# HongMJ1315/Path_Tracing

Hardware: AMD Instinct MI355X
Metric: Msamples/s (paths/s) at 1024^2 x 256spp (higher is better)
Workload: dtype f32; 1 GPU; configs[2]: unidirectional PT + NEE, Cornell-style box + tessellated sphere, 99024 triangles behind a BVH, 1024x1024, 256 spp, depth 4, 1 cone light; parallelism=image tiles 32x32 round-robin over 1 rank(s), RCCL gather to rank 0, seed=1

## Files before the change

### include/hpt.h

```cpp
#ifndef HPT_H
#define HPT_H

#include <stddef.h>
#include <stdint.h>

#ifdef __cplusplus
extern "C" {
#endif

#define HPT_OK 0
#define HPT_ERR_INVALID 1
#define HPT_ERR_DEVICE 2
#define HPT_ERR_NOMEM 3

#define HPT_LIGHT_BYTES 144
#define HPT_SPHERE_BYTES 100
#define HPT_TRIANGLE_BYTES 120
#define HPT_CAMERA_BYTES 84

typedef struct hpt_scene hpt_scene;

typedef struct hpt_params {
    uint64_t seed;
    int32_t sample_offset;
// ... 90 lines not shown
    uint64_t photon_rays;
    uint64_t deposits;
    uint64_t hit_points;
    uint64_t direct_pixels;
    uint64_t candidates;
    uint64_t accepted;
    uint64_t cand_median, cand_max, acc_median, acc_max;
    uint64_t grid_buckets;
    double ms_eye, ms_photon, ms_grid, ms_gather;
    double ms_total;
} hpt_ppm_stats;
int hpt_ppm_get_stats(const hpt_scene *scene, hpt_ppm_stats *out);

int hpt_ppm_render_wrapper(const void *lights, int num_lights, const void *spheres, int num_spheres,
                           const void *triangles, int num_triangles,
                           const float scene_min[3], const float scene_max[3],
                           const void *camera, float *host_image, int W, int H,
                           int light_depth, int light_sample, int eye_depth, int spp, int64_t seed);

typedef struct hpt_sppm hpt_sppm;
int hpt_sppm_create(hpt_scene *scene, const void *camera, int W, int H, int eye_depth, int light_depth, int spl,
                    float radius, float alpha, const float *scene_min, const float *scene_max,
                    const hpt_params *params, hpt_sppm **out);
int hpt_sppm_render(hpt_sppm *state, int passes, int32_t flags, float *host_image);
int hpt_sppm_reset(hpt_sppm *state);
int hpt_sppm_read_state(const hpt_sppm *state, float *radius2, float *photons, int64_t *passes);
void hpt_sppm_destroy(hpt_sppm *state);

typedef struct hpt_multi hpt_multi;
int hpt_multi_create(const void *lights, int num_lights, const void *spheres, int num_spheres,
                     const void *triangles, int num_triangles,
                     const int *device_ids, int num_devices, int exchange, hpt_multi **out);
void hpt_multi_destroy(hpt_multi *multi);
int hpt_multi_num_devices(const hpt_multi *multi);
int hpt_multi_set_groups(hpt_multi *multi, const int32_t *obj_kind, const int32_t *obj_index,
                         const int32_t *obj_group, int num_objects);
int hpt_multi_render_pt(hpt_multi *multi, const void *camera, int W, int H, int eye_depth, int spp,
                        const hpt_params *params, float *host_image);
int hpt_multi_render_bdpt(hpt_multi *multi, const void *camera, int W, int H, int eye_depth, int light_depth,
                          int spp, int spl, const hpt_params *params, float *host_image);
int hpt_multi_get_timing(const hpt_multi *multi, double *render_ms_per_device, double *gather_ms, double *total_ms);
int hpt_wrapper_set_devices(int num_devices);

int hpt_probe_functions(const float *records_in, int n, float *results_out);

int hpt_tonemap(const void *d_linear_rgb, void *d_rgb8, int64_t num_pixels, int bgr, void *hip_stream);
int hpt_tonemap_host(const float *linear_rgb, unsigned char *rgb8, int64_t num_pixels, int bgr);
void hpt_tonemap_table(float thresholds_out[256]);
void hpt_tonemap_reference(const float *linear_rgb, unsigned char *rgb8, int64_t num_pixels, int bgr);

typedef struct hpt_denoise_params {
    int32_t iterations;
    float sigma_color;
    float sigma_normal;
    float sigma_position;
    int32_t flags;
} hpt_denoise_params;
#define HPT_DENOISE_DEMODULATE 1
#define HPT_DENOISE_TIME 2

int hpt_render_guides(hpt_scene *scene, const void *camera, int W, int H, int spp,
                      const hpt_params *params,
                      float *albedo, float *normal, float *position, float *coverage);
int hpt_render_guides_device(hpt_scene *scene, const void *camera, int W, int H, int spp,
                             const hpt_params *params,
                             void *d_albedo, void *d_normal, void *d_position, void *d_coverage);

typedef struct hpt_denoiser hpt_denoiser;
int hpt_denoiser_create(int W, int H, hpt_denoiser **out);
int hpt_denoiser_set_guides(hpt_denoiser *d, const void *d_albedo, const void *d_normal,
                            const void *d_position, const void *d_coverage, void *hip_stream);
int hpt_denoiser_run(hpt_denoiser *d, const void *d_linear_rgb, void *d_out,
                     const hpt_denoise_params *p, void *hip_stream);
int hpt_denoiser_last_ms(const hpt_denoiser *d, double *ms_pack, double *ms_filter);
int hpt_denoiser_level_ms(const hpt_denoiser *d, double *ms_levels, int cap);
void hpt_denoiser_destroy(hpt_denoiser *d);
int hpt_denoise_host(const float *linear_rgb, const float *albedo, const float *normal, const float *position,
                     const float *coverage, float *out, int W, int H, const hpt_denoise_params *p);

#define HPT_ACCUM_MOMENTS 1
typedef struct hpt_accum hpt_accum;
int  hpt_accum_create(int W, int H, int32_t flags, hpt_accum **out);
int  hpt_accum_add(hpt_accum *a, const void *d_frame_rgb, void *d_mean_out, void *hip_stream);
int  hpt_accum_mean(hpt_accum *a, void *d_out, void *hip_stream);
int  hpt_accum_variance(hpt_accum *a, void *d_out, void *hip_stream);
int  hpt_accum_reset(hpt_accum *a, void *hip_stream);
int64_t hpt_accum_count(const hpt_accum *a);
int  hpt_accum_read(hpt_accum *a, float *sum, float *sumsq, int64_t *count);
void hpt_accum_destroy(hpt_accum *a);

#define HPT_DISPLAY_BGR    1
#define HPT_DISPLAY_FLIP_Y 2
typedef struct hpt_display hpt_display;
int  hpt_display_create(int W, int H, hpt_display **out);
int  hpt_display_present(hpt_display *d, const void *d_linear_rgb, const hpt_display *other,
                         void *d_rgb8, int64_t pitch_bytes, int64_t x_offset_bytes, int32_t flags, void *hip_stream);
int  hpt_display_metrics(hpt_display *d, double *rms_prev, double *rms_other,
                         uint64_t *ssd_prev, uint64_t *ssd_other, int64_t *presented);
int  hpt_display_reset(hpt_display *d, void *hip_stream);
void hpt_display_destroy(hpt_display *d);

typedef struct hpt_history hpt_history;
typedef struct hpt_history_params {
    float max_history;
    float plane_tolerance;
    float normal_min;
    int32_t flags;
} hpt_history_params;
int  hpt_history_create(int W, int H, hpt_history **out);
int  hpt_history_advance(hpt_history *h, const void *camera, const void *d_frame_rgb,
                         const void *d_normal, const void *d_position, const void *d_coverage,
                         const hpt_history_params *p, void *d_mean_out, void *hip_stream);
int  hpt_history_metrics(hpt_history *h, uint64_t *kept, uint64_t *restarted, int64_t *frames);
int  hpt_history_read(hpt_history *h, float *mean, float *length, int64_t *frames);
int  hpt_history_reset(hpt_history *h, void *hip_stream);
void hpt_history_destroy(hpt_history *h);
int  hpt_history_check(int W, int H, const void *camera, const void *d_frame_rgb,
                       const void *d_normal, const void *d_position, const void *d_coverage,
                       const hpt_history_params *p, const void *d_mean_out);

#define HPT_HISTORY_MOMENTS 1
int  hpt_history_create_flags(int W, int H, int32_t flags, hpt_history **out);
int  hpt_history_variance(hpt_history *h, const void *d_fallback, float min_length, void *d_variance_out, void *hip_stream);
int  hpt_history_read_moments(hpt_history *h, float *q);
int  hpt_history_variance_check(int W, int H, int32_t create_flags, const void *d_fallback, float min_length,
                                const void *d_variance_out);

typedef struct hpt_guided_params {
    int32_t iterations;
    float sigma_color;
    float sigma_normal;
    float sigma_position;
    int32_t flags;
} hpt_guided_params;
int hpt_denoiser_run_guided(hpt_denoiser *d, const void *d_linear_rgb, const void *d_variance,
                            void *d_out, void *d_variance_out,
                            const hpt_guided_params *p, void *hip_stream);
int hpt_denoiser_estimate_variance(hpt_denoiser *d, const void *d_frame_rgb, const void *d_length,
                                   void *d_variance_out, const hpt_guided_params *p, void *hip_stream);
int hpt_history_length(hpt_history *h, void *d_length_out, void *hip_stream);
int hpt_guided_check(int W, int H, const void *d_linear_rgb, const void *d_variance, const void *d_out,
                     const void *d_variance_out, const hpt_guided_params *p);

typedef struct hpt_bvh_info {
    int32_t num_nodes, num_tris, bvh_depth, num_rounds;
    float qorigin[3], qscale[3];
} hpt_bvh_info;
int hpt_bvh_export_host(const void *lights, int num_lights, const void *spheres, int num_spheres,
                        const void *triangles, int num_triangles, hpt_bvh_info *info,
                        void *qnodes_out, size_t qnodes_cap, void *tris_out, size_t tris_cap);
int hpt_scene_export_bvh(const hpt_scene *scene, hpt_bvh_info *info,
                         void *qnodes_out, size_t qnodes_cap, void *tris_out, size_t tris_cap);

int hpt_trace_closest(hpt_scene *scene, const float *origins, const float *dirs, int n,
                      int flags, float *t_out, int32_t *prim_out);
int hpt_trace_visibility(hpt_scene *scene, const float *p1, const float *p2, int n,
                         int flags, int32_t *visible_out);

typedef struct hpt_update_info {
    uint64_t updates, live_tris, dead_tris;
    double ms_pack, ms_upload, ms_refit;
} hpt_update_info;
int hpt_scene_update_triangles(hpt_scene *scene, const void *triangles, int num_triangles);
int hpt_scene_update_rounds(hpt_scene *scene, const void *lights, int num_lights, const void *spheres, int num_spheres);
int hpt_scene_update_check(const hpt_scene *scene, const void *triangles, int num_triangles);
int hpt_scene_get_update_info(const hpt_scene *scene, hpt_update_info *out);
int hpt_bvh_refit_host(const void *lights, int num_lights, const void *spheres, int num_spheres, const void *triangles,
                       const void *new_triangles, int num_triangles, hpt_bvh_info *info,
                       void *qnodes_out, size_t qnodes_cap, void *tris_out, size_t tris_cap);

#ifdef __cplusplus
}
#endif
#endif
```

### path_tracing_amd/__init__.py

```python
from __future__ import annotations

import ctypes as C
import os

import numpy as np

from . import layouts, scene_io
from .layouts import CAMERA, LIGHT, SPHERE, TRIANGLE

_HERE = os.path.dirname(os.path.abspath(__file__))
LIB_PATH = os.path.join(_HERE, "csrc", "libhpt.so")

FLAG_BRUTE_FORCE = 1
FLAG_COUNT_WORK = 2
FLAG_OUTPUT_SUM = 4
FLAG_TIME_KERNELS = 8
FLAG_RUSSIAN_ROULETTE = 16
FLAG_SINGLE_PIPELINE = 32
FLAG_NO_HOST_WAIT = 64
DENOISE_DEMODULATE = 1
DENOISE_TIME = 2
ACCUM_MOMENTS = 1
DISPLAY_BGR = 1
DISPLAY_FLIP_Y = 2
HISTORY_MOMENTS = 1


class HptError(RuntimeError):
    pass


class Params(C.Structure):
    _fields_ = [("seed", C.c_uint64), ("sample_offset", C.c_int32), ("max_delta", C.c_int32),
                ("rank", C.c_int32), ("world", C.c_int32), ("tile", C.c_int32),
                ("samples_per_pass", C.c_int32), ("flags", C.c_int32), ("reserved", C.c_int32)]


class Stats(C.Structure):
    _fields_ = [("samples", C.c_uint64), ("closest_rays", C.c_uint64), ("shadow_rays", C.c_uint64),
                ("boxes_closest", C.c_uint64), ("tris_closest", C.c_uint64),
                ("boxes_shadow", C.c_uint64), ("tris_shadow", C.c_uint64), ("path_iters", C.c_uint64),
                ("ms_total", C.c_double), ("ms_extend", C.c_double), ("ms_shade", C.c_double),
                ("ms_connect", C.c_double), ("ms_other", C.c_double),
                ("n_extend", C.c_uint32), ("n_shade", C.c_uint32), ("n_connect", C.c_uint32), ("n_other", C.c_uint32),
                ("bvh_nodes", C.c_uint32), ("bvh_depth", C.c_uint32), ("n_tris", C.c_uint32), ("n_materials", C.c_uint32),
                ("ms_bvh_build", C.c_double), ("ms_upload", C.c_double),
                ("lane_steps_closest", C.c_uint64), ("wave_steps_closest", C.c_uint64),
                ("lane_steps_shadow", C.c_uint64), ("wave_steps_shadow", C.c_uint64),
                ("leaf_lane_closest", C.c_uint64), ("leaf_wave_closest", C.c_uint64),
                ("leaf_lane_shadow", C.c_uint64), ("leaf_wave_shadow", C.c_uint64),
                ("ms_resume", C.c_double), ("n_resume", C.c_uint32), ("split_budget", C.c_uint32),
                ("traced_rays_last_pass", C.c_uint64), ("long_rays_last_pass", C.c_uint64),
                ("bd_pairs", C.c_uint64), ("bd_survivors", C.c_uint64), ("bd_shadow_rays", C.c_uint64), ("bd_unoccluded", C.c_uint64),
                ("bd_nodes", C.c_uint64), ("bd_tris", C.c_uint64), ("bd_spheres", C.c_uint64), ("bd_group_boxes", C.c_uint64)]

    def as_dict(self):
        return {n: getattr(self, n) for n, _ in self._fields_}


class PpmStats(C.Structure):
    _fields_ = [(n, C.c_uint64) for n in ("photons", "photon_rays", "deposits", "hit_points", "direct_pixels", "candidates", "accepted",
                                          "cand_median", "cand_max", "acc_median", "acc_max", "grid_buckets")] + \
               [(n, C.c_double) for n in ("ms_eye", "ms_photon", "ms_grid", "ms_gather", "ms_total")]

    def as_dict(self):
        return {n: getattr(self, n) for n, _ in self._fields_}


class DenoiseParams(C.Structure):
    _fields_ = [("iterations", C.c_int32), ("sigma_color", C.c_float), ("sigma_normal", C.c_float),
                ("sigma_position", C.c_float), ("flags", C.c_int32)]


class GuidedParams(C.Structure):
    _fields_ = [("iterations", C.c_int32), ("sigma_color", C.c_float), ("sigma_normal", C.c_float),
                ("sigma_position", C.c_float), ("flags", C.c_int32)]


class HistoryParams(C.Structure):
    _fields_ = [("max_history", C.c_float), ("plane_tolerance", C.c_float), ("normal_min", C.c_float), ("flags", C.c_int32)]


def make_history_params(max_history=0.0, plane_tolerance=0.0, normal_min=0.0) -> HistoryParams:
    return HistoryParams(float(max_history), float(plane_tolerance), float(normal_min), 0)


def make_denoise_params(iterations=0, sigma_color=0.0, sigma_normal=0.0, sigma_position=0.0, demodulate=True, time=False) -> DenoiseParams:
    return DenoiseParams(int(iterations), float(sigma_color), float(sigma_normal), float(sigma_position),
                         (DENOISE_DEMODULATE if demodulate else 0) | (DENOISE_TIME if time else 0))


def make_guided_params(iterations=0, sigma_color=0.0, sigma_normal=0.0, sigma_position=0.0, demodulate=True, time=False) -> GuidedParams:
    return GuidedParams(int(iterations), float(sigma_color), float(sigma_normal), float(sigma_position),
                        (DENOISE_DEMODULATE if demodulate else 0) | (DENOISE_TIME if time else 0))


class BvhInfo(C.Structure):
    _fields_ = [("num_nodes", C.c_int32), ("num_tris", C.c_int32), ("bvh_depth", C.c_int32), ("num_rounds", C.c_int32),
                ("qorigin", C.c_float * 3), ("qscale", C.c_float * 3)]


class UpdateInfo(C.Structure):
    _fields_ = [("updates", C.c_uint64), ("live_tris", C.c_uint64), ("dead_tris", C.c_uint64),
                ("ms_pack", C.c_double), ("ms_upload", C.c_double), ("ms_refit", C.c_double)]


QNODE_WORDS = 8
TRI_WORDS = 12

_lib = None


def _share_the_hip_runtime_with_torch():
    import importlib.util
    import sys
    if "torch" in sys.modules:
        return
    try:
        spec = importlib.util.find_spec("torch")
    except (ImportError, ValueError):
        spec = None
    if spec and spec.origin:
        cand = os.path.join(os.path.dirname(spec.origin), "lib", "libamdhip64.so")
        if os.path.exists(cand):
            C.CDLL(cand, mode=C.RTLD_GLOBAL)


def load_library() -> C.CDLL:
    global _lib
    if _lib is None:
        _share_the_hip_runtime_with_torch()
        path = os.environ.get("HPT_LIBRARY") or LIB_PATH
        if not os.path.exists(path):
            raise HptError("%s not built: run `make -C path_tracing_amd/csrc` "
                           "(or __graft_entry__.build()); there is no CPU fallback" % path)
        lib = C.CDLL(path)
        lib.hpt_last_error.restype = C.c_char_p
        lib.hpt_local_pixels.restype = C.c_int64
        lib.hpt_local_pixels.argtypes = [C.c_int, C.c_int, C.POINTER(Params)]
        for name in ("hpt_scene_create", "hpt_render_pt", "hpt_render_pt_device", "hpt_untile", "hpt_scene_set_groups",
                     "hpt_render_bdpt", "hpt_render_bdpt_device", "hpt_bdpt_render_wrapper",
                     "hpt_pt_render_wrapper", "hpt_get_stats", "hpt_trace_closest", "hpt_trace_visibility",
                     "hpt_device_count", "hpt_multi_create", "hpt_multi_num_devices", "hpt_multi_set_groups",
                     "hpt_multi_render_pt", "hpt_multi_render_bdpt", "hpt_multi_get_timing", "hpt_wrapper_set_devices",
                     "hpt_probe_functions", "hpt_tonemap", "hpt_tonemap_host", "hpt_bvh_export_host", "hpt_scene_export_bvh",
                     "hpt_render_ppm", "hpt_ppm_get_stats", "hpt_ppm_render_wrapper",
                     "hpt_sppm_create", "hpt_sppm_render", "hpt_sppm_reset", "hpt_sppm_read_state",
                     "hpt_render_guides", "hpt_denoiser_create", "hpt_denoiser_set_guides", "hpt_denoiser_run",
                     "hpt_denoiser_last_ms", "hpt_denoiser_level_ms", "hpt_denoise_host",
                     "hpt_accum_create", "hpt_accum_add", "hpt_accum_mean", "hpt_accum_variance", "hpt_accum_reset", "hpt_accum_read",
                     "hpt_display_create", "hpt_display_present", "hpt_display_metrics", "hpt_display_reset",
                     "hpt_render_guides_device", "hpt_history_create", "hpt_history_advance", "hpt_history_metrics",
                     "hpt_history_read", "hpt_history_reset", "hpt_history_check",
                     "hpt_denoiser_run_guided", "hpt_denoiser_estimate_variance", "hpt_history_length", "hpt_guided_check",
                     "hpt_history_create_flags", "hpt_history_variance", "hpt_history_read_moments", "hpt_history_variance_check",
                     "hpt_scene_update_triangles", "hpt_scene_update_rounds", "hpt_scene_update_check", "hpt_scene_get_update_info",
                     "hpt_bvh_refit_host"):
            if hasattr(lib, name):
                getattr(lib, name).restype = C.c_int
        if hasattr(lib, "hpt_sppm_destroy"):
            lib.hpt_sppm_destroy.restype = None
            lib.hpt_sppm_destroy.argtypes = [C.c_void_p]
        if hasattr(lib, "hpt_denoiser_destroy"):
            lib.hpt_denoiser_destroy.restype = None
            lib.hpt_denoiser_destroy.argtypes = [C.c_void_p]
        for name in ("hpt_accum_destroy", "hpt_display_destroy", "hpt_history_destroy"):
            if hasattr(lib, name):
                getattr(lib, name).restype = None
                getattr(lib, name).argtypes = [C.c_void_p]
        if hasattr(lib, "hpt_accum_count"):
            lib.hpt_accum_count.restype = C.c_int64
            lib.hpt_accum_count.argtypes = [C.c_void_p]
        lib.hpt_scene_destroy.restype = None
        lib.hpt_wrapper_cache_clear.restype = None
        lib.hpt_wrapper_cache_clear.argtypes = []
        lib.hpt_scene_destroy.argtypes = [C.c_void_p]
        lib.hpt_multi_destroy.restype = None
        lib.hpt_multi_destroy.argtypes = [C.c_void_p]
        _lib = lib
    return _lib


def _check(rc: int):
    if rc != 0:
        raise HptError("hpt error %d: %s" % (rc, load_library().hpt_last_error().decode("utf-8", "replace")))


def _vp(a):
    return a.ctypes.data_as(C.c_void_p) if a is not None and a.size else None


def device_count() -> int:
    return int(load_library().hpt_device_count())


def make_params(seed=1, sample_offset=0, max_delta=0, rank=0, world=1, tile=0, samples_per_pass=0, flags=0) -> Params:
    p = Params()
    p.seed, p.sample_offset, p.max_delta = int(seed), int(sample_offset), int(max_delta)
    p.rank, p.world, p.tile, p.samples_per_pass, p.flags, p.reserved = rank, world, tile, samples_per_pass, flags, 0
    return p


def local_pixels(W: int, H: int, params: Params) -> int:
    n = int(load_library().hpt_local_pixels(W, H, C.byref(params)))
    if n < 0:
        _check(1)
    return n


class Scene:

    def __init__(self, lights, spheres, triangles):
        self._lib = load_library()
        self._h = C.c_void_p()
        lights = np.ascontiguousarray(lights, LIGHT)
        spheres = np.ascontiguousarray(spheres, SPHERE)
        triangles = np.ascontiguousarray(triangles, TRIANGLE)
        _check(self._lib.hpt_scene_create(_vp(lights), len(lights), _vp(spheres), len(spheres),
                                          _vp(triangles), len(triangles), C.byref(self._h)))
        self.num_lights, self.num_spheres, self.num_triangles = len(lights), len(spheres), len(triangles)

    def close(self):
        if getattr(self, "_h", None) is not None and self._h:
            self._lib.hpt_scene_destroy(self._h)
            self._h = C.c_void_p()

    def __del__(self):
        try:
            self.close()
        except Exception:
            pass

    def __enter__(self):
        return self

    def __exit__(self, *exc):
        self.close()

    def render_pt(self, camera, W, H, eye_depth=4, spp=8, params: Params | None = None) -> np.ndarray:
        params = params or make_params()
        cam = np.ascontiguousarray(camera, CAMERA)
        img = np.empty((H, W, 3), np.float32)
        _check(self._lib.hpt_render_pt(self._h, _vp(cam.reshape(1)), W, H, eye_depth, spp, C.byref(params), _vp(img)))
        return img

    def render_pt_device(self, camera, W, H, eye_depth, spp, params: Params, d_local_ptr: int, stream: int = 0):
        cam = np.ascontiguousarray(camera, CAMERA)
        _check(self._lib.hpt_render_pt_device(self._h, _vp(cam.reshape(1)), W, H, eye_depth, spp, C.byref(params),
                                              C.c_void_p(d_local_ptr), C.c_void_p(stream)))

    def set_groups(self, kind, index, group):
        k = np.ascontiguousarray(kind, np.int32); i = np.ascontiguousarray(index, np.int32); g = np.ascontiguousarray(group, np.int32)
        _check(self._lib.hpt_scene_set_groups(self._h, _vp(k), _vp(i), _vp(g), len(k)))

    def render_bdpt(self, camera, W, H, eye_depth=4, light_depth=4, spp=8, spl=8, params: Params | None = None) -> np.ndarray:
        params = params or make_params()
        cam = np.ascontiguousarray(camera, CAMERA)
        img = np.empty((H, W, 3), np.float32)
        _check(self._lib.hpt_render_bdpt(self._h, _vp(cam.reshape(1)), W, H, eye_depth, light_depth, spp, spl, C.byref(params), _vp(img)))
        return img

    def render_bdpt_device(self, camera, W, H, eye_depth, light_depth, spp, spl, params: Params, d_local_ptr: int, stream: int = 0):
        cam = np.ascontiguousarray(camera, CAMERA)
        _check(self._lib.hpt_render_bdpt_device(self._h, _vp(cam.reshape(1)), W, H, eye_depth, light_depth, spp, spl, C.byref(params),
                                                C.c_void_p(d_local_ptr), C.c_void_p(stream)))

    def render_ppm(self, camera, W, H, eye_depth=4, light_depth=4, spp=1, spl=8, radius=0.05, params: Params | None = None,
                   scene_min=None, scene_max=None) -> np.ndarray:
        params = params or make_params()
        cam = np.ascontiguousarray(camera, CAMERA)
        img = np.empty((H, W, 3), np.float32)
        mn = (C.c_float * 3)(*scene_min) if scene_min is not None else None
        mx = (C.c_float * 3)(*scene_max) if scene_max is not None else None
        _check(self._lib.hpt_render_ppm(self._h, _vp(cam.reshape(1)), W, H, eye_depth, light_depth, spp, spl, C.c_float(radius),
                                        mn, mx, C.byref(params), _vp(img)))
        return img

    def ppm_stats(self) -> dict:
        st = PpmStats()
        _check(self._lib.hpt_ppm_get_stats(self._h, C.byref(st)))
        return st.as_dict()

    def sppm(self, camera, W, H, eye_depth=4, light_depth=4, spl=8, radius=0.05, alpha=0.7, params: Params | None = None,
             scene_min=None, scene_max=None) -> "Sppm":
        return Sppm(self, camera, W, H, eye_depth, light_depth, spl, radius, alpha, params, scene_min, scene_max)

    def render_guides(self, camera, W, H, spp=4, params: Params | None = None) -> dict:
        params = params or make_params()
        cam = np.ascontiguousarray(camera, CAMERA)
        g = dict(albedo=np.empty((H, W, 3), np.float32), normal=np.empty((H, W, 3), np.float32),
                 position=np.empty((H, W, 3), np.float32), coverage=np.empty((H, W), np.float32))
        _check(self._lib.hpt_render_guides(self._h, _vp(cam.reshape(1)), W, H, int(spp), C.byref(params), _vp(g["albedo"]),
                                           _vp(g["normal"]), _vp(g["position"]), _vp(g["coverage"])))
        return g

    def render_guides_device(self, camera, W, H, spp=4, params: Params | None = None, albedo=None, normal=None, position=None,
                             coverage=None):
        params = params or make_params()
        cam = np.ascontiguousarray(camera, CAMERA)
        ptr = [_dptr(x) if x is not None else None for x in (albedo, normal, position, coverage)]
        _check(self._lib.hpt_render_guides_device(self._h, _vp(cam.reshape(1)), W, H, int(spp), C.byref(params), *ptr))

    def stats(self) -> dict:
        st = Stats()
        _check(self._lib.hpt_get_stats(self._h, C.byref(st)))
        return st.as_dict()

    def export_bvh(self) -> dict:
        return _export_bvh(lambda info, qn, qcap, tr, tcap: self._lib.hpt_scene_export_bvh(self._h, info, qn, qcap, tr, tcap))

# ... 253 lines not shown
    def __init__(self, W, H, moments=False):
        self._lib = load_library()
        self._h = C.c_void_p()
        self.W, self.H, self.moments = int(W), int(H), bool(moments)
        if moments:
            _check(self._lib.hpt_history_create_flags(int(W), int(H), C.c_int32(HISTORY_MOMENTS), C.byref(self._h)))
        else:
            _check(self._lib.hpt_history_create(int(W), int(H), C.byref(self._h)))

    def advance(self, camera, frame, normal=None, position=None, coverage=None, params: HistoryParams | None = None, mean_out=None,
                stream: int = 0):
        cam = np.ascontiguousarray(camera, CAMERA)
        opt = [_dptr(x) if x is not None else None for x in (normal, position, coverage)]
        _check(self._lib.hpt_history_advance(self._h, _vp(cam.reshape(1)), _dptr(frame), opt[0], opt[1], opt[2],
                                             C.byref(params) if params is not None else None,
                                             _dptr(mean_out) if mean_out is not None else None, C.c_void_p(stream)))

    def metrics(self) -> dict:
        k, r = C.c_uint64(), C.c_uint64()
        n = C.c_int64()
        _check(self._lib.hpt_history_metrics(self._h, C.byref(k), C.byref(r), C.byref(n)))
        return dict(kept=int(k.value), restarted=int(r.value), frames=int(n.value))

    def read(self) -> dict:
        m = np.empty((self.H, self.W, 3), np.float32)
        n = np.empty((self.H, self.W), np.float32)
        k = C.c_int64()
        _check(self._lib.hpt_history_read(self._h, _vp(m), _vp(n), C.byref(k)))
        out = dict(mean=m, length=n, frames=int(k.value))
        if self.moments:
            q = np.empty((self.H, self.W, 3), np.float32)
            _check(self._lib.hpt_history_read_moments(self._h, _vp(q)))
            out["q"] = q
        return out

    def variance(self, out, fallback=None, min_length=0.0, stream: int = 0):
        _check(self._lib.hpt_history_variance(self._h, _dptr(fallback) if fallback is not None else None, C.c_float(min_length),
                                              _dptr(out) if out is not None else None, C.c_void_p(stream)))

    def length(self, out, stream: int = 0):
        _check(self._lib.hpt_history_length(self._h, _dptr(out), C.c_void_p(stream)))

    def reset(self, stream: int = 0):
        _check(self._lib.hpt_history_reset(self._h, C.c_void_p(stream)))

    def close(self):
        if getattr(self, "_h", None) is not None and self._h:
            self._lib.hpt_history_destroy(self._h)
            self._h = C.c_void_p()

    def __del__(self):
        try:
            self.close()
        except Exception:
            pass

    def __enter__(self):
        return self

    def __exit__(self, *exc):
        self.close()


class MultiScene:

    def __init__(self, lights, spheres, triangles, device_ids=None, num_devices=0, exchange=0):
        self._lib = load_library()
        self._h = C.c_void_p()
        lights = np.ascontiguousarray(lights, LIGHT)
        spheres = np.ascontiguousarray(spheres, SPHERE)
        triangles = np.ascontiguousarray(triangles, TRIANGLE)
        ids = None
        if device_ids is not None:
            ids = np.ascontiguousarray(device_ids, np.int32)
            num_devices = len(ids)
        _check(self._lib.hpt_multi_create(_vp(lights), len(lights), _vp(spheres), len(spheres), _vp(triangles), len(triangles),
                                          _vp(ids), int(num_devices), int(exchange), C.byref(self._h)))
        self.num_devices = int(self._lib.hpt_multi_num_devices(self._h))

    def close(self):
        if getattr(self, "_h", None) is not None and self._h:
            self._lib.hpt_multi_destroy(self._h)
            self._h = C.c_void_p()

    def __del__(self):
        try:
            self.close()
        except Exception:
            pass

    def __enter__(self):
        return self

    def __exit__(self, *exc):
        self.close()

    def set_groups(self, kind, index, group):
        k = np.ascontiguousarray(kind, np.int32); i = np.ascontiguousarray(index, np.int32); g = np.ascontiguousarray(group, np.int32)
        _check(self._lib.hpt_multi_set_groups(self._h, _vp(k), _vp(i), _vp(g), len(k)))

    def render_pt(self, camera, W, H, eye_depth=4, spp=8, params: Params | None = None) -> np.ndarray:
        params = params or make_params()
        cam = np.ascontiguousarray(camera, CAMERA)
        img = np.empty((H, W, 3), np.float32)
        _check(self._lib.hpt_multi_render_pt(self._h, _vp(cam.reshape(1)), W, H, eye_depth, spp, C.byref(params), _vp(img)))
        return img

    def render_bdpt(self, camera, W, H, eye_depth=4, light_depth=4, spp=8, spl=8, params: Params | None = None) -> np.ndarray:
        params = params or make_params()
        cam = np.ascontiguousarray(camera, CAMERA)
        img = np.empty((H, W, 3), np.float32)
        _check(self._lib.hpt_multi_render_bdpt(self._h, _vp(cam.reshape(1)), W, H, eye_depth, light_depth, spp, spl, C.byref(params), _vp(img)))
        return img

    def timing(self) -> dict:
        per = (C.c_double * self.num_devices)()
        g = C.c_double(); t = C.c_double()
        _check(self._lib.hpt_multi_get_timing(self._h, per, C.byref(g), C.byref(t)))
        return {"render_ms_per_device": list(per), "gather_ms": g.value, "total_ms": t.value}


def _export_bvh(call) -> dict:
    info = BvhInfo()
    _check(call(C.byref(info), None, C.c_size_t(0), None, C.c_size_t(0)))
    qn = np.zeros((max(info.num_nodes, 1), QNODE_WORDS), np.uint32)
    tr = np.zeros((max(info.num_tris, 1), TRI_WORDS), np.uint32)
    _check(call(C.byref(info), _vp(qn), C.c_size_t(qn.nbytes), _vp(tr), C.c_size_t(tr.nbytes)))
    return {"num_nodes": info.num_nodes, "num_tris": info.num_tris, "bvh_depth": info.bvh_depth, "num_rounds": info.num_rounds,
            "qorigin": np.array(info.qorigin, np.float32), "qscale": np.array(info.qscale, np.float32),
            "qnodes": qn[:info.num_nodes], "tris": tr[:info.num_tris]}


def export_bvh_host(lights, spheres, triangles) -> dict:
    lib = load_library()
    lights = np.ascontiguousarray(lights, LIGHT)
    spheres = np.ascontiguousarray(spheres, SPHERE)
    triangles = np.ascontiguousarray(triangles, TRIANGLE)
    return _export_bvh(lambda info, qn, qcap, tr, tcap: lib.hpt_bvh_export_host(
        _vp(lights), len(lights), _vp(spheres), len(spheres), _vp(triangles), len(triangles), info, qn, qcap, tr, tcap))


def refit_bvh_host(lights, spheres, triangles, new_triangles) -> dict:
    lib = load_library()
    lights = np.ascontiguousarray(lights, LIGHT)
    spheres = np.ascontiguousarray(spheres, SPHERE)
    triangles = np.ascontiguousarray(triangles, TRIANGLE)
    new_triangles = np.ascontiguousarray(new_triangles, TRIANGLE)
    if len(new_triangles) != len(triangles):
        raise HptError("hpt error 1: an update keeps the triangle count: %d triangles, %d were handed over" % (len(triangles), len(new_triangles)))
    return _export_bvh(lambda info, qn, qcap, tr, tcap: lib.hpt_bvh_refit_host(
        _vp(lights), len(lights), _vp(spheres), len(spheres), _vp(triangles), _vp(new_triangles), len(triangles), info, qn, qcap, tr, tcap))


def update_check(scene, triangles, num_triangles=None) -> None:
    tr = np.ascontiguousarray(triangles, TRIANGLE) if triangles is not None else None
    n = len(tr) if num_triangles is None else int(num_triangles)
    _check(load_library().hpt_scene_update_check(scene._h if scene is not None else None, _vp(tr) if tr is not None else None, n))


def probe_functions(records) -> np.ndarray:
    rec = np.ascontiguousarray(records, np.float32).reshape(-1, 24)
    out = np.zeros((len(rec), 40), np.float32)
    _check(load_library().hpt_probe_functions(_vp(rec), len(rec), _vp(out)))
    return out


def tonemap(image) -> np.ndarray:
    img = np.ascontiguousarray(image, np.float32)
    out = np.zeros(img.shape, np.uint8)
    _check(load_library().hpt_tonemap_host(_vp(img), _vp(out), C.c_int64(img.size // 3), 0))
    return out


def tonemap_device(d_linear_rgb, d_rgb8, num_pixels: int, bgr: bool = False, stream: int = 0):
    _check(load_library().hpt_tonemap(_dptr(d_linear_rgb), _dptr(d_rgb8), C.c_int64(num_pixels), 1 if bgr else 0, C.c_void_p(stream)))


def wrapper_set_devices(n: int) -> None:
    _check(load_library().hpt_wrapper_set_devices(int(n)))


def untile(d_gathered_ptr: int, d_image_ptr: int, W: int, H: int, params: Params, stream: int = 0):
    _check(load_library().hpt_untile(C.c_void_p(d_gathered_ptr), C.c_void_p(d_image_ptr), W, H, C.byref(params), C.c_void_p(stream)))


def wrapper_cache_clear() -> None:
    load_library().hpt_wrapper_cache_clear()


def pt_render_wrapper(lights, spheres, triangles, camera, W, H, eye_depth, spp, seed=-1,
                      scene_min=(0, 0, 0), scene_max=(0, 0, 0), light_depth=4, light_sample=8) -> np.ndarray:
    lib = load_library()
    lights = np.ascontiguousarray(lights, LIGHT)
    spheres = np.ascontiguousarray(spheres, SPHERE)
    triangles = np.ascontiguousarray(triangles, TRIANGLE)
    cam = np.ascontiguousarray(camera, CAMERA).reshape(1)
    img = np.empty((H, W, 3), np.float32)
    mn = (C.c_float * 3)(*scene_min)
    mx = (C.c_float * 3)(*scene_max)
    _check(lib.hpt_pt_render_wrapper(_vp(lights), len(lights), _vp(spheres), len(spheres), _vp(triangles), len(triangles),
                                     mn, mx, _vp(cam), _vp(img), W, H, light_depth, light_sample, eye_depth, spp,
                                     C.c_int64(seed)))
    return img


def ppm_render_wrapper(lights, spheres, triangles, camera, W, H, scene_min, scene_max, light_depth=4, light_sample=8,
                       eye_depth=4, spp=1, seed=-1) -> np.ndarray:
    lib = load_library()
    lights = np.ascontiguousarray(lights, LIGHT)
    spheres = np.ascontiguousarray(spheres, SPHERE)
    triangles = np.ascontiguousarray(triangles, TRIANGLE)
    cam = np.ascontiguousarray(camera, CAMERA).reshape(1)
    img = np.empty((H, W, 3), np.float32)
    mn = (C.c_float * 3)(*scene_min)
    mx = (C.c_float * 3)(*scene_max)
    _check(lib.hpt_ppm_render_wrapper(_vp(lights), len(lights), _vp(spheres), len(spheres), _vp(triangles), len(triangles),
                                      mn, mx, _vp(cam), _vp(img), W, H, light_depth, light_sample, eye_depth, spp, C.c_int64(seed)))
    return img
```

### path_tracing_amd/csrc/hpt_api.cpp

```cpp
#include "hpt_host.h"

#include <chrono>
#include <cmath>
#include <cstdio>
#include <cstdlib>
#include <ctime>
#include <mutex>
#include <new>

using namespace hpt;

static_assert(sizeof(hpt_stats) == 312 && sizeof(hpt_params) == 40, "ABI records: keep path_tracing_amd/__init__.py and tests/test_boundary.py in step");

namespace {

thread_local std::string g_err;

}

namespace hpt {

int fail(int code, const std::string &msg){ g_err = msg; return code; }

int make_tiling(int W, int H, const hpt_params *p, Tiling &tl){
// ... 43 lines not shown
    HIP_TRY(s->ws.local_own.reserve((size_t) tl.n_local * 3));
    HIP_TRY(s->ws.image_own.reserve((size_t) tl.W * tl.H * 3));
    return HPT_OK;
}

int untile_to_host(hpt_scene *s, const Tiling &tl, hipStream_t st, float *host_image, hipEvent_t after){
    launch_untile(st, tl, s->ws.local_own.get(), s->ws.image_own.get());
    if(after) HIP_TRY(hipEventRecord(after, st));
    HIP_TRY(hipGetLastError());
    HIP_TRY(hipMemcpy(host_image, s->ws.image_own.get(), (size_t) tl.W * tl.H * 3 * sizeof(float), hipMemcpyDeviceToHost));
    return HPT_OK;
}

}

namespace {

int collect_stats(hpt_scene *s){
    if(!s->tm.stats_pending) return HPT_OK;
    HIP_TRY(hipEventSynchronize(s->tm.ev_stop));
    float ms = 0.f;
    HIP_TRY(hipEventElapsedTime(&ms, s->tm.ev_start, s->tm.ev_stop));
    s->tm.stats.ms_total = ms;
    double sum[5] = { 0, 0, 0, 0, 0 }; uint32_t cnt[5] = { 0, 0, 0, 0, 0 };
    for(const TimedLaunch &t : s->tm.timed){
        float e = 0.f;
        if(hipEventElapsedTime(&e, t.a, t.b) == hipSuccess){ sum[t.cls] += e; cnt[t.cls]++; }
    }
    s->tm.stats.ms_extend = sum[0]; s->tm.stats.ms_shade = sum[1]; s->tm.stats.ms_connect = sum[2]; s->tm.stats.ms_other = sum[3];
    s->tm.stats.n_extend = cnt[0]; s->tm.stats.n_shade = cnt[1]; s->tm.stats.n_connect = cnt[2]; s->tm.stats.n_other = cnt[3];
    s->tm.stats.ms_resume = sum[4]; s->tm.stats.n_resume = cnt[4];
    s->tm.stats.split_budget = (uint32_t) s->ws.last_budget;
    s->tm.stats.traced_rays_last_pass = s->tm.stats.long_rays_last_pass = 0;
    if(s->ws.last_counter_stride > 0 && s->ws.last_counters){
        std::vector<uint32_t> h((size_t) 4 * s->ws.last_counter_stride);
        HIP_TRY(hipMemcpy(h.data(), s->ws.last_counters, h.size() * sizeof(uint32_t), hipMemcpyDeviceToHost));
        for(int i = 0; i < s->ws.last_counter_stride; ++i){
            s->tm.stats.traced_rays_last_pass += (uint64_t) h[i] + h[(size_t) s->ws.last_counter_stride + i];
            s->tm.stats.long_rays_last_pass += (uint64_t) h[(size_t) 2 * s->ws.last_counter_stride + i] + h[(size_t) 3 * s->ws.last_counter_stride + i];
        }
    }
    WorkCounters wc;
    HIP_TRY(hipMemcpy(&wc, s->ws.wc.get(), sizeof wc, hipMemcpyDeviceToHost));
    s->tm.stats.samples = wc.samples; s->tm.stats.closest_rays = wc.closest_rays; s->tm.stats.shadow_rays = wc.shadow_rays;
    s->tm.stats.boxes_closest = wc.boxes_closest; s->tm.stats.tris_closest = wc.tris_closest;
    s->tm.stats.boxes_shadow = wc.boxes_shadow; s->tm.stats.tris_shadow = wc.tris_shadow; s->tm.stats.path_iters = wc.path_iters;
    s->tm.stats.lane_steps_closest = wc.lane_steps_closest; s->tm.stats.wave_steps_closest = wc.wave_steps_closest;
    s->tm.stats.lane_steps_shadow = wc.lane_steps_shadow; s->tm.stats.wave_steps_shadow = wc.wave_steps_shadow;
    s->tm.stats.leaf_lane_closest = wc.leaf_lane_closest; s->tm.stats.leaf_wave_closest = wc.leaf_wave_closest;
    s->tm.stats.leaf_lane_shadow = wc.leaf_lane_shadow; s->tm.stats.leaf_wave_shadow = wc.leaf_wave_shadow;
    s->tm.stats.bd_pairs = wc.bd_pairs; s->tm.stats.bd_survivors = wc.bd_survivors; s->tm.stats.bd_shadow_rays = wc.bd_shadow_rays;
    s->tm.stats.bd_unoccluded = wc.bd_unoccluded; s->tm.stats.bd_nodes = wc.bd_nodes; s->tm.stats.bd_tris = wc.bd_tris;
    s->tm.stats.bd_spheres = wc.bd_spheres; s->tm.stats.bd_group_boxes = wc.bd_group_boxes;
    s->tm.stats_pending = false;
    return HPT_OK;
}

struct WrapperCache { std::mutex mu; hpt_scene *scene = nullptr; int device = -1; hpt_multi *multi = nullptr; int devices = 0; } g_wrap;

bool wrapper_cache_enabled(){
    static const bool on = [](){ const char *e = getenv("HPT_WRAPPER_CACHE"); return !(e && e[0] == '0'); }();
    return on;
}

int wrapper_devices(){
    if(g_wrap.devices > 0) return g_wrap.devices;
    static const int from_env = [](){ const char *e = getenv("HPT_DEVICES"); int v = e ? atoi(e) : 1; return v > 0 ? v : 1; }();
    return from_env;
}

int wrapper_scene(const void *lights, int nl, const void *spheres, int ns, const void *tris, int nt, hpt_scene **out){
    int dev = -1;
    if(hipGetDevice(&dev) != hipSuccess) dev = -1;
    hpt_scene *k = g_wrap.scene;
    if(k && wrapper_cache_enabled() && dev == g_wrap.device && nl == k->geo.nl && ns == k->geo.ns && nt == k->geo.nt && nl >= 0 && ns >= 0 && nt >= 0 &&
       same_bytes(k->geo.h_lights, lights, (size_t) nl * HPT_LIGHT_BYTES) && same_bytes(k->geo.h_spheres, spheres, (size_t) ns * HPT_SPHERE_BYTES) &&
       same_bytes(k->geo.h_tris, tris, (size_t) nt * HPT_TRIANGLE_BYTES)){
        *out = k;
        return HPT_OK;
    }
    if(k){ hpt_scene_destroy(k); g_wrap.scene = nullptr; g_wrap.device = -1; }
    int rc = hpt_scene_create(lights, nl, spheres, ns, tris, nt, out);
    if(rc) return rc;
    if(wrapper_cache_enabled()){ g_wrap.scene = *out; g_wrap.device = dev; }
    return HPT_OK;
}

void wrapper_release(hpt_scene *s){
    if(s == g_wrap.scene) return;
    std::string keep = g_err;
    hpt_scene_destroy(s);
    g_err = keep;
}

int wrapper_multi(int devices, const void *lights, int nl, const void *spheres, int ns, const void *tris, int nt, hpt_multi **out){
    if(g_wrap.multi && wrapper_cache_enabled() && hpt::multi_matches(g_wrap.multi, devices, lights, nl, spheres, ns, tris, nt)){
        *out = g_wrap.multi;
        return HPT_OK;
    }
    if(g_wrap.multi){ hpt_multi_destroy(g_wrap.multi); g_wrap.multi = nullptr; }
    int rc = hpt_multi_create(lights, nl, spheres, ns, tris, nt, nullptr, devices, 0, out);
    if(rc) return rc;
    if(wrapper_cache_enabled()) g_wrap.multi = *out;
    return HPT_OK;
}

void wrapper_release_multi(hpt_multi *m){
    if(m == g_wrap.multi) return;
    std::string keep = g_err;
    hpt_multi_destroy(m);
    g_err = keep;
}

hpt_params wrapper_params(int64_t seed){
    hpt_params p; memset(&p, 0, sizeof p);
    p.seed = seed >= 0 ? (uint64_t) seed : (uint64_t) time(nullptr);
    return p;
}

template <typename One, typename Many>
int wrapper_render(const void *lights, int nl, const void *spheres, int ns, const void *tris, int nt, One one, Many many){
    std::lock_guard<std::mutex> lock(g_wrap.mu);
    if(wrapper_devices() > 1){
        hpt_multi *m = nullptr;
        int rc = wrapper_multi(wrapper_devices(), lights, nl, spheres, ns, tris, nt, &m);
        if(rc) return rc;
        rc = many(m);
        wrapper_release_multi(m);
        return rc;
    }
    hpt_scene *s = nullptr;
    int rc = wrapper_scene(lights, nl, spheres, ns, tris, nt, &s);
    if(rc) return rc;
    rc = one(s);
    wrapper_release(s);
    return rc;
}

}

namespace hpt {

int scene_upload(const HostScene &hs, const void *lights, int nl, const void *spheres, int ns, const void *tris, int nt,
                 hpt_scene **out){
    *out = nullptr;
    hpt_scene *s = new (std::nothrow) hpt_scene();
    if(!s) return fail(HPT_ERR_NOMEM, "out of host memory");
    auto t0 = std::chrono::steady_clock::now();
    hipError_t e = hipGetDevice(&s->device);
    if(e == hipSuccess){ hipDeviceProp_t prop; if(hipGetDeviceProperties(&prop, s->device) == hipSuccess && prop.multiProcessorCount > 0) s->num_cus = prop.multiProcessorCount; }
    if(e == hipSuccess) e = s->geo.nodes.upload(hs.nodes);
    if(e == hipSuccess) e = s->geo.qnodes.upload(hs.qnodes);
    if(e == hipSuccess) e = s->geo.wnodes.upload(hs.wnodes);
    if(e == hipSuccess) e = s->geo.tris.upload(hs.tris);
    if(e == hipSuccess) e = s->geo.rounds.upload(hs.rounds);
    if(e == hipSuccess) e = s->geo.mats.upload(hs.materials);
    if(e == hipSuccess) e = s->geo.lights.upload(hs.lights);
    if(e != hipSuccess){ hpt_scene_destroy(s); return fail_hip("scene upload", e); }
    e = s->geo.tri_frames.reserve(std::max<size_t>((size_t) nt, 1) * 4);
    if(e == hipSuccess){
        launch_tri_frames(nullptr, (const float4 *) s->geo.tris.get(), nt, s->geo.tri_frames.get());
        e = hipDeviceSynchronize();
    }
    if(e != hipSuccess){ hpt_scene_destroy(s); return fail_hip("triangle frames", e); }
    auto t1 = std::chrono::steady_clock::now();
    s->geo.sd.nodes = (const float4 *) s->geo.nodes.get(); s->geo.sd.tris = (const float4 *) s->geo.tris.get();
    s->geo.sd.tri_frames = s->geo.tri_frames.get();
    s->geo.sd.qnodes = (const uint4 *) s->geo.qnodes.get();
    s->geo.sd.wnodes = (const uint4 *) s->geo.wnodes.get(); s->geo.sd.wide_depth = hs.wide_depth;
    for(int a = 0; a < 3; ++a){ s->geo.sd.qorigin[a] = hs.qorigin[a]; s->geo.sd.qscale[a] = hs.qscale[a]; }
    s->geo.sd.rounds = s->geo.rounds.get(); s->geo.sd.mats = s->geo.mats.get(); s->geo.sd.lights = s->geo.lights.get();
    s->geo.sd.num_rounds = ns + nl; s->geo.sd.num_spheres = ns; s->geo.sd.num_lights = nl; s->geo.sd.num_tris = nt;
    s->geo.sd.num_mats = (int) hs.materials.size(); s->geo.sd.num_nodes = (int) hs.qnodes.size();
    s->geo.nl = nl; s->geo.ns = ns; s->geo.nt = nt;
    if(nl) s->geo.h_lights.assign((const unsigned char *) lights, (const unsigned char *) lights + (size_t) nl * HPT_LIGHT_BYTES);
    if(ns) s->geo.h_spheres.assign((const unsigned char *) spheres, (const unsigned char *) spheres + (size_t) ns * HPT_SPHERE_BYTES);
    if(nt) s->geo.h_tris.assign((const unsigned char *) tris, (const unsigned char *) tris + (size_t) nt * HPT_TRIANGLE_BYTES);
    memset(&s->tm.stats, 0, sizeof s->tm.stats);
    s->tm.stats.bvh_nodes = (uint32_t) hs.nodes.size(); s->tm.stats.bvh_depth = (uint32_t) hs.bvh_depth;
    s->geo.stack_levels = hs.bvh_depth > 0 ? hs.bvh_depth : 1;
    s->tm.stats.n_tris = (uint32_t) nt; s->tm.stats.n_materials = (uint32_t) hs.materials.size();
    s->tm.stats.ms_bvh_build = hs.ms_bvh_build;
    s->tm.stats.ms_upload = std::chrono::duration<double, std::milli>(t1 - t0).count();
    s->up.level_begin = hs.level_begin; s->up.wide_src = hs.wide_src; s->up.num_wide = (uint32_t) hs.wnodes.size();
    s->up.sphere_material.resize((size_t) ns);
    for(int i = 0; i < ns; ++i) s->up.sphere_material[(size_t) i] = hs.rounds[(size_t) i].material;
    *out = s;
    return HPT_OK;
}

int export_host_tree(const HostScene &hs, hpt_bvh_info *info, void *qnodes_out, size_t qnodes_cap, void *tris_out, size_t tris_cap){
    info->num_nodes = (int32_t) hs.qnodes.size(); info->num_tris = (int32_t) hs.tris.size();
    info->bvh_depth = hs.bvh_depth; info->num_rounds = hs.num_spheres + hs.num_lights;
    for(int a = 0; a < 3; ++a){ info->qorigin[a] = hs.qorigin[a]; info->qscale[a] = hs.qscale[a]; }
    if(qnodes_out){
        if(qnodes_cap < hs.qnodes.size() * sizeof(QBvhNode)) return fail(HPT_ERR_INVALID, "qnodes_out too small");
        memcpy(qnodes_out, hs.qnodes.data(), hs.qnodes.size() * sizeof(QBvhNode));
    }
    if(tris_out){
        if(tris_cap < hs.tris.size() * sizeof(DevTriangle)) return fail(HPT_ERR_INVALID, "tris_out too small");
        memcpy(tris_out, hs.tris.data(), hs.tris.size() * sizeof(DevTriangle));
    }
    return HPT_OK;
}

}

extern "C" {

const char *hpt_last_error(void){ return g_err.c_str(); }

int hpt_device_count(void){
    int n = 0;
    if(hipGetDeviceCount(&n) != hipSuccess) return -1;
    return n;
}

int hpt_scene_create(const void *lights, int nl, const void *spheres, int ns, const void *tris, int nt,
                     hpt_scene **out){
    if(!out) return fail(HPT_ERR_INVALID, "null out_scene");
    *out = nullptr;
    HostScene hs;
    const char *err = build_host_scene(lights, nl, spheres, ns, tris, nt, hs);
    if(err && *err) return fail(HPT_ERR_INVALID, err);
    return hpt::scene_upload(hs, lights, nl, spheres, ns, tris, nt, out);
}

void hpt_scene_destroy(hpt_scene *s){
    if(!s) return;
    for(PassBuffers &w : s->ws.pass) if(w.h_count) hipHostFree(w.h_count);
    if(s->ws.px_fork) hipEventDestroy(s->ws.px_fork);
    for(int k = 1; k < kMaxPipes; ++k){
        if(s->ws.px_done[k]) hipEventDestroy(s->ws.px_done[k]);
        if(s->ws.px_stream[k]) hipStreamDestroy(s->ws.px_stream[k]);
    }
    for(hipEvent_t e : s->pm.marks) hipEventDestroy(e);
    if(s->up.ev_a) hipEventDestroy(s->up.ev_a);
    if(s->up.ev_b) hipEventDestroy(s->up.ev_b);
    if(s->tm.ev_start) hipEventDestroy(s->tm.ev_start);
    if(s->tm.ev_stop) hipEventDestroy(s->tm.ev_stop);
    for(hipEvent_t e : s->tm.event_pool) hipEventDestroy(e);
    delete s;
}

int64_t hpt_local_pixels(int W, int H, const hpt_params *params){
    Tiling tl;
    if(make_tiling(W, H, params, tl)) return -1;
    return tl.n_local;
}

int hpt_untile(const void *d_gathered, void *d_image, int W, int H, const hpt_params *params, void *hip_stream){
    Tiling tl;
    int rc = make_tiling(W, H, params, tl);
    if(rc) return rc;
    if(!d_gathered || !d_image) return fail(HPT_ERR_INVALID, "null buffer");
    launch_untile((hipStream_t) hip_stream, tl, (const float *) d_gathered, (float *) d_image);
    HIP_TRY(hipGetLastError());
    return HPT_OK;
}


void hpt_wrapper_cache_clear(void){
    std::lock_guard<std::mutex> lock(g_wrap.mu);
    if(g_wrap.scene) hpt_scene_destroy(g_wrap.scene);
    g_wrap.scene = nullptr; g_wrap.device = -1;
    if(g_wrap.multi) hpt_multi_destroy(g_wrap.multi);
    g_wrap.multi = nullptr;
}

int hpt_wrapper_set_devices(int num_devices){
    if(num_devices < 0) return fail(HPT_ERR_INVALID, "negative device count");
    std::lock_guard<std::mutex> lock(g_wrap.mu);
    g_wrap.devices = num_devices;
    return HPT_OK;
}

int hpt_pt_render_wrapper(const void *lights, int nl, const void *spheres, int ns, const void *tris, int nt,
                          const float scene_min[3], const float scene_max[3], const void *camera, float *host_image,
                          int W, int H, int light_depth, int light_sample, int eye_depth, int spp, int64_t seed){
    (void) scene_min; (void) scene_max; (void) light_depth; (void) light_sample;
    const hpt_params p = wrapper_params(seed);
    return wrapper_render(lights, nl, spheres, ns, tris, nt,
        [&](hpt_scene *s){ return hpt_render_pt(s, camera, W, H, eye_depth, spp, &p, host_image); },
        [&](hpt_multi *m){ return hpt_multi_render_pt(m, camera, W, H, eye_depth, spp, &p, host_image); });
}

namespace {

unsigned char tonemap_byte(float x){
    float c = std::max(0.0f, std::min(x, 1.0f));
    float g = std::pow(c, 1.0f / 2.2f);
    return (unsigned char) (g * 255.0f);
}

const float *tonemap_thresholds(){
    static float table[256];
    static std::once_flag once;
    std::call_once(once, [](){
        table[0] = -INFINITY;
        for(int k = 1; k < 256; ++k){
            uint32_t lo = 0u, hi = 0x3F800000u;
            while(lo < hi){
                uint32_t mid = lo + (hi - lo) / 2u;
                float x; memcpy(&x, &mid, 4);
                if((int) tonemap_byte(x) >= k) hi = mid; else lo = mid + 1u;
            }
            memcpy(&table[k], &lo, 4);
        }
    });
    return table;
}

struct TonemapDevice { std::mutex mu; DevBuf<float> table[64]; } &g_tonemap = *new TonemapDevice;

int tonemap_device_table(const float **out){
    int dev = 0;
    HIP_TRY(hipGetDevice(&dev));
    if(dev < 0 || dev >= 64) return fail(HPT_ERR_INVALID, "device ordinal out of range");
    std::lock_guard<std::mutex> lock(g_tonemap.mu);
    DevBuf<float> &d = g_tonemap.table[dev];
    if(!d.get()){
        HIP_TRY(d.reserve(256));
        hipError_t e = hipMemcpy(d.get(), tonemap_thresholds(), 256 * sizeof(float), hipMemcpyHostToDevice);
        if(e != hipSuccess){ d.release(); return fail(HPT_ERR_DEVICE, std::string("tonemap table upload: ") + hipGetErrorString(e)); }
    }
    *out = d.get();
    return HPT_OK;
}

}

void hpt_tonemap_table(float thresholds_out[256]){ memcpy(thresholds_out, tonemap_thresholds(), 256 * sizeof(float)); }

void hpt_tonemap_reference(const float *linear_rgb, unsigned char *rgb8, int64_t num_pixels, int bgr){
    for(int64_t p = 0; p < num_pixels; ++p)
        for(int c = 0; c < 3; ++c) rgb8[p * 3 + c] = tonemap_byte(linear_rgb[p * 3 + (bgr ? 2 - c : c)]);
}

int hpt_tonemap(const void *d_linear_rgb, void *d_rgb8, int64_t num_pixels, int bgr, void *hip_stream){
    if(num_pixels < 0 || (num_pixels > 0 && (!d_linear_rgb || !d_rgb8))) return fail(HPT_ERR_INVALID, "bad tonemap argument");
    if(((uintptr_t) d_rgb8 & 3u) != 0u) return fail(HPT_ERR_INVALID, "tonemap output must be 4-byte aligned");
    const float *table = nullptr;
    int rc = tonemap_device_table(&table);
    if(rc) return rc;
    launch_tonemap((hipStream_t) hip_stream, (const float *) d_linear_rgb, d_rgb8, (unsigned long long) num_pixels * 3ull, bgr ? 1 : 0, table);
    HIP_TRY(hipGetLastError());
    return HPT_OK;
}

int hpt_tonemap_host(const float *linear_rgb, unsigned char *rgb8, int64_t num_pixels, int bgr){
    if(num_pixels < 0 || (num_pixels > 0 && (!linear_rgb || !rgb8))) return fail(HPT_ERR_INVALID, "bad tonemap argument");
    if(num_pixels == 0) return HPT_OK;
    DevBuf<float> d_in; DevBuf<unsigned char> d_out;
    size_t n = (size_t) num_pixels * 3;
    HIP_TRY(d_in.reserve(n));
    HIP_TRY(d_out.reserve((n + 3) / 4 * 4));
    HIP_TRY(hipMemcpy(d_in.get(), linear_rgb, n * sizeof(float), hipMemcpyHostToDevice));
    int rc = hpt_tonemap(d_in.get(), d_out.get(), num_pixels, bgr, nullptr);
    if(rc) return rc;
    HIP_TRY(hipMemcpy(rgb8, d_out.get(), n, hipMemcpyDeviceToHost));
    return HPT_OK;
}

int hpt_get_stats(const hpt_scene *scene, hpt_stats *out){
    if(!scene || !out) return fail(HPT_ERR_INVALID, "null argument");
    int rc = collect_stats(const_cast<hpt_scene *>(scene));
    if(rc) return rc;
    *out = scene->tm.stats;
    return HPT_OK;
}

int hpt_trace_closest(hpt_scene *s, const float *origins, const float *dirs, int n, int flags,
                      float *t_out, int32_t *prim_out){
    if(!s || !origins || !dirs || !t_out || !prim_out || n < 0) return fail(HPT_ERR_INVALID, "bad argument");
    if(n == 0) return HPT_OK;
    DevBuf<float> d_o, d_d, d_t; DevBuf<int32_t> d_p;
    size_t b3 = (size_t) n * 3 * sizeof(float);
    HIP_TRY(d_o.reserve((size_t) n * 3)); HIP_TRY(d_d.reserve((size_t) n * 3));
    HIP_TRY(d_t.reserve((size_t) n)); HIP_TRY(d_p.reserve((size_t) n));
    HIP_TRY(hipMemcpy(d_o.get(), origins, b3, hipMemcpyHostToDevice));
    HIP_TRY(hipMemcpy(d_d.get(), dirs, b3, hipMemcpyHostToDevice));
    launch_probe_closest(nullptr, s->geo.sd, d_o.get(), d_d.get(), n, (flags & HPT_FLAG_BRUTE_FORCE) ? 1 : 0, d_t.get(), d_p.get());
    HIP_TRY(hipGetLastError());
    HIP_TRY(hipMemcpy(t_out, d_t.get(), (size_t) n * 4, hipMemcpyDeviceToHost));
    HIP_TRY(hipMemcpy(prim_out, d_p.get(), (size_t) n * 4, hipMemcpyDeviceToHost));
    return HPT_OK;
}

int hpt_probe_functions(const float *records_in, int n, float *results_out){
    if(n < 0 || (n > 0 && (!records_in || !results_out))) return fail(HPT_ERR_INVALID, "bad argument");
    if(n == 0) return HPT_OK;
    DevBuf<float> d_in, d_out;
    HIP_TRY(d_in.reserve((size_t) n * 24));
    HIP_TRY(d_out.reserve((size_t) n * 40));
    HIP_TRY(hipMemcpy(d_in.get(), records_in, (size_t) n * 24 * sizeof(float), hipMemcpyHostToDevice));
    launch_probe_functions(nullptr, d_in.get(), n, d_out.get());
    HIP_TRY(hipGetLastError());
    HIP_TRY(hipMemcpy(results_out, d_out.get(), (size_t) n * 40 * sizeof(float), hipMemcpyDeviceToHost));
    return HPT_OK;
}

int hpt_scene_set_groups(hpt_scene *s, const int32_t *obj_kind, const int32_t *obj_index, const int32_t *obj_group, int nobj){
    if(!s) return fail(HPT_ERR_INVALID, "null scene");
    if(nobj < 0 || (nobj > 0 && (!obj_kind || !obj_index || !obj_group))) return fail(HPT_ERR_INVALID, "bad group arrays");
    if(nobj != 0 && nobj != s->geo.ns + s->geo.nt) return fail(HPT_ERR_INVALID, "group arrays must list every sphere and triangle once");
    s->geo.g_kind.assign(obj_kind, obj_kind + nobj); s->geo.g_index.assign(obj_index, obj_index + nobj); s->geo.g_group.assign(obj_group, obj_group + nobj);
    s->bd.ready = false;
    return HPT_OK;
}


int hpt_bdpt_render_wrapper(const void *lights, int nl, const void *spheres, int ns, const void *tris, int nt,
                            const float scene_min[3], const float scene_max[3], const void *camera, float *host_image,
                            int W, int H, int light_depth, int light_sample, int eye_depth, int spp, int spl, int64_t seed){
    (void) scene_min; (void) scene_max;
    std::vector<unsigned char> L((const unsigned char *) lights, (const unsigned char *) lights + (size_t) std::max(nl, 0) * HPT_LIGHT_BYTES);
    if(light_sample > 1) for(int i = 0; i < nl; ++i){
        float *illum = (float *) (L.data() + (size_t) i * HPT_LIGHT_BYTES + 24);
        for(int c = 0; c < 3; ++c) illum[c] = illum[c] * (float) light_sample;
    }
    const hpt_params p = wrapper_params(seed);
    return wrapper_render(L.data(), nl, spheres, ns, tris, nt,
        [&](hpt_scene *s){ return hpt_render_bdpt(s, camera, W, H, eye_depth, light_depth, spp, spl, &p, host_image); },
        [&](hpt_multi *m){ return hpt_multi_render_bdpt(m, camera, W, H, eye_depth, light_depth, spp, spl, &p, host_image); });
}

int hpt_ppm_render_wrapper(const void *lights, int nl, const void *spheres, int ns, const void *tris, int nt,
                           const float scene_min[3], const float scene_max[3], const void *camera, float *host_image,
                           int W, int H, int light_depth, int light_sample, int eye_depth, int spp, int64_t seed){
    (void) spp;
    std::lock_guard<std::mutex> lock(g_wrap.mu);
    hpt_scene *s = nullptr;
    int rc = wrapper_scene(lights, nl, spheres, ns, tris, nt, &s);
    if(rc) return rc;
    const hpt_params p = wrapper_params(seed);
    rc = hpt_render_ppm(s, camera, W, H, eye_depth, light_depth, 1, light_sample, 0.05f, scene_min, scene_max, &p, host_image);
    wrapper_release(s);
    return rc;
}

int hpt_bvh_export_host(const void *lights, int nl, const void *spheres, int ns, const void *tris, int nt, hpt_bvh_info *info,
                        void *qnodes_out, size_t qnodes_cap, void *tris_out, size_t tris_cap){
    if(!info) return fail(HPT_ERR_INVALID, "null info");
    HostScene hs;
    const char *err = build_host_scene(lights, nl, spheres, ns, tris, nt, hs);
    if(err && *err) return fail(HPT_ERR_INVALID, err);
    return export_host_tree(hs, info, qnodes_out, qnodes_cap, tris_out, tris_cap);
}

int hpt_scene_export_bvh(const hpt_scene *s, hpt_bvh_info *info, void *qnodes_out, size_t qnodes_cap, void *tris_out, size_t tris_cap){
    if(!s || !info) return fail(HPT_ERR_INVALID, "null argument");
    if(int rcd = on_scene_device(s)) return rcd;
    info->num_nodes = s->geo.sd.num_nodes; info->num_tris = s->geo.sd.num_tris;
    info->bvh_depth = (int32_t) s->tm.stats.bvh_depth; info->num_rounds = s->geo.sd.num_rounds;
    for(int a = 0; a < 3; ++a){ info->qorigin[a] = s->geo.sd.qorigin[a]; info->qscale[a] = s->geo.sd.qscale[a]; }
    if(qnodes_out){
        const size_t bytes = (size_t) s->geo.sd.num_nodes * sizeof(QBvhNode);
        if(qnodes_cap < bytes) return fail(HPT_ERR_INVALID, "qnodes_out too small");
        HIP_TRY(hipMemcpy(qnodes_out, s->geo.qnodes.get(), bytes, hipMemcpyDeviceToHost));
    }
    if(tris_out){
        const size_t bytes = (size_t) s->geo.sd.num_tris * sizeof(DevTriangle);
        if(tris_cap < bytes) return fail(HPT_ERR_INVALID, "tris_out too small");
        if(bytes) HIP_TRY(hipMemcpy(tris_out, s->geo.tris.get(), bytes, hipMemcpyDeviceToHost));
    }
    return HPT_OK;
}

int hpt_trace_visibility(hpt_scene *s, const float *p1, const float *p2, int n, int flags, int32_t *vis_out){
    if(!s || !p1 || !p2 || !vis_out || n < 0) return fail(HPT_ERR_INVALID, "bad argument");
    if(n == 0) return HPT_OK;
    DevBuf<float> d_a, d_b; DevBuf<int32_t> d_v;
    size_t b3 = (size_t) n * 3 * sizeof(float);
    HIP_TRY(d_a.reserve((size_t) n * 3)); HIP_TRY(d_b.reserve((size_t) n * 3));
    HIP_TRY(d_v.reserve((size_t) n));
    HIP_TRY(hipMemcpy(d_a.get(), p1, b3, hipMemcpyHostToDevice));
    HIP_TRY(hipMemcpy(d_b.get(), p2, b3, hipMemcpyHostToDevice));
    launch_probe_visibility(nullptr, s->geo.sd, d_a.get(), d_b.get(), n, (flags & HPT_FLAG_BRUTE_FORCE) ? 1 : 0, d_v.get());
    HIP_TRY(hipGetLastError());
    HIP_TRY(hipMemcpy(vis_out, d_v.get(), (size_t) n * 4, hipMemcpyDeviceToHost));
    return HPT_OK;
}

}
```

### path_tracing_amd/csrc/hpt_host.h

```cpp
#pragma once
#include "../../include/hpt.h"
#include "hpt_scene.h"
#include "pt_kernels.h"
#include "bdpt_kernels.h"
#include "ppm_kernels.h"
#include "denoise_kernels.h"
#include "refit_kernels.h"

#include <hip/hip_runtime.h>
#include <algorithm>
#include <cstring>
#include <string>
#include <vector>

namespace hpt {

int fail(int code, const std::string &msg);

inline int fail_hip(const std::string &what, hipError_t e){
    return fail(e == hipErrorOutOfMemory ? HPT_ERR_NOMEM : HPT_ERR_DEVICE, what + ": " + hipGetErrorString(e));
}

#define HIP_TRY(expr) do { hipError_t e_ = (expr); if(e_ != hipSuccess) return hpt::fail_hip(#expr, e_); } while(0)

template <typename T>
class DevBuf {
    T *p_ = nullptr; size_t cap_ = 0;
public:
    DevBuf() = default;
    DevBuf(const DevBuf &) = delete;
    DevBuf &operator=(const DevBuf &) = delete;
    ~DevBuf(){ release(); }
    T *get() const { return p_; }
    size_t capacity() const { return cap_; }
    void release(){ if(p_) hipFree(p_); p_ = nullptr; cap_ = 0; }
    hipError_t reserve(size_t n){
        if(n <= cap_) return hipSuccess;
        release();
        hipError_t e = hipMalloc((void **) &p_, n * sizeof(T));
        if(e != hipSuccess){ p_ = nullptr; return e; }
        cap_ = n;
        return hipSuccess;
    }
    template <typename A>
    hipError_t upload(const std::vector<T, A> &v){
        release();
        hipError_t e = reserve(std::max<size_t>(v.size(), 1));
        if(e == hipSuccess && !v.empty()) e = hipMemcpy(p_, v.data(), v.size() * sizeof(T), hipMemcpyHostToDevice);
        return e;
    }
};

template <typename First, typename... Rest>
hipError_t reserve_all(size_t n, First &first, Rest &... rest){
    if(n <= first.capacity()) return hipSuccess;
    first.release(); (rest.release(), ...);
    hipError_t e = first.reserve(n);
    ((e = e == hipSuccess ? rest.reserve(n) : e), ...);
    if(e != hipSuccess){ first.release(); (rest.release(), ...); }
    return e;
}

struct TimedLaunch { hipEvent_t a, b; int cls; };
constexpr int kMaxPipes = 2;

}

struct hpt_scene {
    int device = 0;
    int num_cus = 256;

    struct Geometry {
        hpt::SceneDev sd{};
        hpt::DevBuf<hpt::BvhNode> nodes; hpt::DevBuf<hpt::QBvhNode> qnodes; hpt::DevBuf<hpt::WideNode> wnodes;
        hpt::DevBuf<hpt::DevTriangle> tris; hpt::DevBuf<hpt::DevRound> rounds;
        hpt::DevBuf<hpt::DevMaterial> mats; hpt::DevBuf<hpt::DevLight> lights;
        hpt::DevBuf<float4> tri_frames;
        int stack_levels = hpt::kStackDepth;
        std::vector<unsigned char> h_lights, h_spheres, h_tris;
        int nl = 0, ns = 0, nt = 0;
        std::vector<int32_t> g_kind, g_index, g_group;
    } geo;

    struct PassBuffers {
        hpt::DevBuf<float4> org_eta, dir_flags, thr, col; hpt::DevBuf<uint2> rng, hit;
        hpt::DevBuf<float4> org_max, dir, contrib;
        hpt::PathBuf pb{}; hpt::ShadowBuf sb{};
        hpt::DevBuf<uint32_t> queue[2];
        hpt::DevBuf<uint32_t> squeue;
        hpt::DevBuf<uint32_t> lqueue[2];
        hpt::DevBuf<hpt::DeferredRay> rec;
        hpt::DevBuf<uint32_t> deep_stack;
        hpt::DevBuf<uint32_t> counters;
        uint32_t *h_count = nullptr;
        size_t cap_paths() const { return org_eta.capacity(); }
    };
    struct Workspace {
        PassBuffers pass[hpt::kMaxPipes];
        hipStream_t px_stream[hpt::kMaxPipes] = {}; int px_priority[hpt::kMaxPipes] = {};
        hipEvent_t px_fork = nullptr, px_done[hpt::kMaxPipes] = {};
        const uint32_t *last_counters = nullptr;
        int last_counter_stride = 0;
        int last_budget = 0;
        hpt::DevBuf<float4> accum;
        hpt::DevBuf<hpt::WorkCounters> wc;
        hpt::DevBuf<float> local_own, image_own;
    } ws;

    struct Bdpt {
        bool ready = false;
        hpt::BdptSceneDev sc{};
        hpt::DevBuf<hpt::BvhNode> nodes; hpt::DevBuf<hpt::DevTriangle> tris; hpt::DevBuf<hpt::DevRound> spheres;
        hpt::DevBuf<hpt::DevGroup> groups; hpt::DevBuf<hpt::DevMaterial> mats; hpt::DevBuf<hpt::DevLight> lights;
        hpt::DevBuf<float4> last_pos_pdf, last_normal, vtx_pos, vtx_nrm, vtx_thr, vtx_wo, vtx_base, ectx, hist_pos_eta, contrib;
        hpt::DevBuf<float2> hist_pdf; hpt::DevBuf<unsigned long long> valid;
        hpt::BdptPathBuf bp{};
        hpt::DevBuf<hpt::LightVertexDev> lv; hpt::DevBuf<hpt::LightVertexCtx> lctx; hpt::DevBuf<uint32_t> cqueue;
    } bd;

    struct Ppm {
        bool bounds_ready = false; float min[3] = {0, 0, 0}, max[3] = {0, 0, 0};
        hpt::DevBuf<float4> pos_mat, nrm, wo, thr; hpt::DevBuf<uint32_t> list;
        hpt::DevBuf<float4> dep, packed; hpt::DevBuf<uint32_t> key, slot_in, key_sorted, slot_sorted;
        hpt::DevBuf<uint2> range; hpt::DevBuf<unsigned char> sort_tmp;
        hpt::PpmHitBuf hb{}; hpt::PpmGrid grid{};
        hpt::DevBuf<uint32_t> cand, acc;
        hpt::DevBuf<hpt::PpmCounters> pc;
        hpt::DevBuf<float4> g_alb, g_nrm, g_pos;
        std::vector<hipEvent_t> marks;
        hpt_ppm_stats stats{};
    } pm;

    struct Update {
        std::vector<uint32_t> level_begin;
        hpt::pod_vector<uint32_t> wide_src;
        std::vector<uint32_t> sphere_material;
        uint32_t num_wide = 0;
        bool ready = false;
        hpt::DevBuf<uint4> d_wide_src;
        hpt::DevBuf<float> verts, slot_box, exact, partial, result;
        std::vector<float> h_verts;
        hipEvent_t ev_a = nullptr, ev_b = nullptr;
        hpt_update_info info{};
    } up;

    struct Timing {
        hipEvent_t ev_start = nullptr, ev_stop = nullptr;
        std::vector<hpt::TimedLaunch> timed; std::vector<hipEvent_t> event_pool; size_t event_next = 0;
        hpt_stats stats{};
        bool stats_pending = false;
    } tm;
};

namespace hpt {

using PassBuffers = hpt_scene::PassBuffers;


int on_scene_device(const hpt_scene *s);

struct ParamRules {
    const char *one_device;
    int32_t flags; const char *flags_msg;
    int32_t reserved; const char *reserved_msg;
};
constexpr int32_t kKnownFlags = HPT_FLAG_BRUTE_FORCE | HPT_FLAG_COUNT_WORK | HPT_FLAG_OUTPUT_SUM | HPT_FLAG_TIME_KERNELS |
                                HPT_FLAG_RUSSIAN_ROULETTE | HPT_FLAG_SINGLE_PIPELINE | HPT_FLAG_NO_HOST_WAIT;
constexpr int32_t kReservedBudgetBits = 0x3F << 1;
constexpr ParamRules kRenderParams{ nullptr, kKnownFlags, nullptr, kReservedBudgetBits, nullptr };
int take_params(const hpt_params *params, const ParamRules &rules, hpt_params &P);

int make_tiling(int W, int H, const hpt_params *p, Tiling &tl);

inline void set_camera(CameraDev &cam, const void *camera){
    const float *cf = (const float *) camera;
    memcpy(cam.eye, cf + 0, 12); memcpy(cam.UL, cf + 12, 12); memcpy(cam.dx, cf + 15, 12); memcpy(cam.dy, cf + 18, 12);
}

int ensure_workspace(hpt_scene *s, size_t paths, size_t n_local, int n_counters);

int ensure_own_image(hpt_scene *s, const Tiling &tl);
int untile_to_host(hpt_scene *s, const Tiling &tl, hipStream_t st, float *host_image, hipEvent_t after = nullptr);

inline void reset_render_stats(hpt_scene *s){
    s->tm.timed.clear(); s->tm.event_next = 0;
    s->ws.last_counter_stride = 0; s->ws.last_budget = 0;
    s->tm.stats.ms_total = s->tm.stats.ms_extend = s->tm.stats.ms_shade = s->tm.stats.ms_connect = s->tm.stats.ms_other = 0.0;
    s->tm.stats.n_extend = s->tm.stats.n_shade = s->tm.stats.n_connect = s->tm.stats.n_other = 0;
}

inline hipEvent_t pool_event(hpt_scene *s){
    if(s->tm.event_next == s->tm.event_pool.size()){
        hipEvent_t e; hipEventCreate(&e); s->tm.event_pool.push_back(e);
    }
    return s->tm.event_pool[s->tm.event_next++];
}

struct LaunchTimer {
    hpt_scene *s; hipStream_t st; bool on; TimedLaunch tl;
    LaunchTimer(hpt_scene *s_, hipStream_t st_, bool on_, int cls) : s(s_), st(st_), on(on_) {
        if(on){ tl.a = pool_event(s); tl.b = pool_event(s); tl.cls = cls; hipEventRecord(tl.a, st); }
    }
    ~LaunchTimer(){ if(on){ hipEventRecord(tl.b, st); s->tm.timed.push_back(tl); } }
};

inline bool same_bytes(const std::vector<unsigned char> &kept, const void *given, size_t bytes){
    return kept.size() == bytes && (bytes == 0 || memcmp(kept.data(), given, bytes) == 0);
}

int export_host_tree(const HostScene &hs, hpt_bvh_info *info, void *qnodes_out, size_t qnodes_cap, void *tris_out, size_t tris_cap);

bool multi_matches(const hpt_multi *m, int n_devices, const void *lights, int nl, const void *spheres, int ns, const void *tris, int nt);

}
```

### path_tracing_amd/csrc/hpt_scene.h

```cpp
#pragma once
#include <cstdint>
#include <memory>
#include <utility>
#include <vector>

namespace hpt {

constexpr uint32_t kLeafFlag = 0x80000000u;
constexpr uint32_t kEmptyChild = 0xFFFFFFFFu;
constexpr int kMaxLeafTris = 2;
constexpr int kMaxBvhDepth = 30;
constexpr int kStackDepth = 32;

struct Float4 { float x, y, z, w; };

template <typename T>
struct default_init_allocator : std::allocator<T> {
    template <typename U> struct rebind { using other = default_init_allocator<U>; };
    default_init_allocator() = default;
    template <typename U> default_init_allocator(const default_init_allocator<U> &){}
    template <typename U> void construct(U *p){ ::new((void *) p) U; }
    template <typename U, typename... A> void construct(U *p, A &&... a){ ::new((void *) p) U(std::forward<A>(a)...); }
};
template <typename T> using pod_vector = std::vector<T, default_init_allocator<T>>;

struct BvhNode {
    float lmin[3]; uint32_t left;
    float lmax[3]; uint32_t right;
    float rmin[3]; uint32_t pad0;
    float rmax[3]; uint32_t pad1;
};

struct QBvhNode {
    uint16_t plane[3][2][2];
    uint32_t left, right;
};

struct WideNode { uint32_t w[16]; };

struct DevTriangle {
    float v0[3]; uint32_t ordinal;
    float e1[3]; uint32_t material;
    float e2[3]; uint32_t flags;
};

struct DevRound {
    float c[3]; float r;
    uint32_t material;
    uint32_t flags;
    uint32_t pad[2];
};

struct DevMaterial {
    float base[3]; float roughness;
    float metallic; float eta; uint32_t type; uint32_t pad;
    float diffuse[3]; float pad2;
};

struct DevLight {
    float pos[3]; float r;
    float main_dir[3]; float cos_cutoff;
    float neg_dir[3]; float cutoff;
    float illum[3]; float area;
    uint32_t is_parallel; float cone_ratio;
    uint32_t pad[2];
    float raw_dir[3]; uint32_t pad2;
    float ball_c[3]; uint32_t pad3;
};

static_assert(sizeof(BvhNode) == 64 && sizeof(DevTriangle) == 48 && sizeof(DevRound) == 32, "layout");
static_assert(sizeof(QBvhNode) == 32 && sizeof(WideNode) == 64, "layout");
static_assert(sizeof(DevMaterial) == 48 && sizeof(DevLight) == 112, "layout");

struct HostScene {
    pod_vector<BvhNode> nodes;
    pod_vector<QBvhNode> qnodes;
    pod_vector<WideNode> wnodes;
    int wide_depth = 0;
    pod_vector<uint32_t> wide_src;
    std::vector<uint32_t> level_begin;
    float qorigin[3] = {0, 0, 0}, qscale[3] = {1, 1, 1};
    pod_vector<DevTriangle> tris;
    std::vector<DevRound> rounds;
    std::vector<DevMaterial> materials;
    std::vector<DevLight> lights;
    int num_spheres = 0, num_lights = 0, num_tris = 0;
    int bvh_depth = 0;
    double ms_bvh_build = 0.0;
};

struct DevGroup {
    float mn[3]; uint32_t root;
    float mx[3]; uint32_t sphere_first;
    uint32_t sphere_count; uint32_t pad[3];
};
static_assert(sizeof(DevGroup) == 48, "layout");

struct HostBdptScene {
    std::vector<BvhNode> nodes;
    std::vector<DevTriangle> tris;
    std::vector<DevRound> spheres;
    std::vector<DevGroup> groups;
    std::vector<DevMaterial> materials;
    std::vector<DevLight> lights;
    float scene_min[3], scene_max[3];
    int bvh_depth = 0;
};

const char *build_bdpt_host_scene(const void *lights, int nl, const void *spheres, int ns, const void *tris, int nt,
                                  const int32_t *obj_kind, const int32_t *obj_index, const int32_t *obj_group, int nobj,
                                  HostBdptScene &out);

const char *build_host_scene(const void *lights, int nl, const void *spheres, int ns,
                             const void *tris, int nt, HostScene &out);


const char *flatten_rounds_host(const void *lights, int nl, const void *spheres, int ns, const uint32_t *sphere_material,
                                std::vector<DevRound> &rounds, std::vector<DevLight> &lights_out);

const char *check_triangle_update(const void *kept, int kept_nt, const void *tris, int nt, char *msg, size_t msg_cap);
const char *check_rounds_update(const void *kept_spheres, int kept_ns, int kept_nl, const void *lights, int nl, const void *spheres, int ns,
                                char *msg, size_t msg_cap);

const char *refit_host_scene(HostScene &hs, const void *tris, int nt, uint64_t *dead_out = nullptr);

float box_padding_of(const float scene_min[3], const float scene_max[3], int nt);
void grid_of_box(const float lo[3], const float hi[3], float qorigin[3], float qscale[3]);

}

struct hpt_scene;
namespace hpt {
int scene_upload(const HostScene &hs, const void *lights, int nl, const void *spheres, int ns, const void *tris, int nt,
                 hpt_scene **out);
}
```

### path_tracing_amd/csrc/pt_kernels.h

```cpp
#pragma once
#include <hip/hip_runtime.h>
#include <cstdint>
#include "hpt_scene.h"

namespace hpt {

struct SceneDev {
    const float4 *nodes;
    const uint4 *qnodes;
    const uint4 *wnodes;
    int wide_depth;
    float qorigin[3], qscale[3];
    const float4 *tris;
    const float4 *tri_frames;
    const DevRound *rounds;
    const DevMaterial *mats;
    const DevLight *lights;
    int num_rounds, num_spheres, num_lights, num_tris, num_mats, num_nodes;
};

struct PathBuf {
    float4 *org_eta;
    float4 *dir_flags;
    float4 *thr;
    float4 *col;
    uint2 *rng;
    uint2 *hit;
};

struct ShadowBuf {
    float4 *org_max;
    float4 *dir;
    float4 *contrib;
};

struct Tiling {
    int W, H, tile, tiles_x, tiles_y, ntiles, rank, world;
    int n_local;
};

struct CameraDev { float eye[3], UL[3], dx[3], dy[3]; };

struct PrimaryGen { Tiling tl; CameraDev cam; uint32_t first_sample; uint32_t pad; uint64_t seed; };

struct WorkCounters {
    unsigned long long boxes_closest, tris_closest, boxes_shadow, tris_shadow, closest_rays, shadow_rays, path_iters, samples,
                       lane_steps_closest, wave_steps_closest, lane_steps_shadow, wave_steps_shadow,
                       leaf_lane_closest, leaf_wave_closest, leaf_lane_shadow, leaf_wave_shadow,
                       bd_pairs, bd_survivors, bd_shadow_rays, bd_unoccluded, bd_nodes, bd_tris, bd_spheres, bd_group_boxes;
};

constexpr uint32_t kHitMiss = 0xFFFFFFFFu;
constexpr uint32_t kHitRoundFlag = 0x80000000u;

constexpr int kBlock = 256;
constexpr uint32_t kLongChunk = 4096;
constexpr int kResumeLdsLevels = 12;
constexpr uint32_t kResumeMaxGroups = 8192;
constexpr int kDeepLevels = 48;
constexpr int kWideRefillMin = 24;
constexpr int kWideNodeMin = 16;
#ifndef HPT_TRACE_BUDGET
#define HPT_TRACE_BUDGET 6
#endif
#ifndef HPT_TOP_LEVELS
#define HPT_TOP_LEVELS 6
#endif
constexpr int kTraceBudget = HPT_TRACE_BUDGET;
constexpr int kTopLevels = HPT_TOP_LEVELS;
constexpr int kTopNodes = 1 << kTopLevels;

void launch_generate(hipStream_t s, const Tiling &tl, const CameraDev &cam, PathBuf pb,
                     uint32_t *qcount, int samples_this_pass, uint32_t first_sample, uint64_t seed,
                     WorkCounters *wc);
void launch_extend(hipStream_t s, const SceneDev &sc, PathBuf pb, const uint32_t *queue, const uint32_t *qcount,
                   uint32_t max_items, int flags, WorkCounters *wc);
void launch_shade(hipStream_t s, const SceneDev &sc, PathBuf pb, const uint32_t *queue, const uint32_t *qcount,
                  uint32_t max_items, uint32_t *next_queue, uint32_t *next_count, ShadowBuf sb, uint32_t *squeue,
                  uint32_t *scount, int max_depth, int max_delta, int roulette, WorkCounters *wc, const PrimaryGen *primary = nullptr,
                  uint32_t max_groups = 0);
void launch_connect(hipStream_t s, const SceneDev &sc, PathBuf pb, ShadowBuf sb, const uint32_t *squeue,
                    const uint32_t *scount, uint32_t max_items, int flags, WorkCounters *wc);
struct DeferredRay {
    float4 org_t;
    float4 dir_slot;
    uint4 hit;
};
struct TraceSplit { uint32_t *equeue, *ecount, *squeue, *scount; int budget; DeferredRay *rec; };
void launch_trace(hipStream_t s, const SceneDev &sc, PathBuf pb, ShadowBuf sb, const uint32_t *equeue,
                  const uint32_t *ecount, uint32_t max_extend, const uint32_t *squeue, const uint32_t *scount,
                  uint32_t max_shadow, int stack_levels, bool count, WorkCounters *wc,
                  const TraceSplit *split = nullptr, const PrimaryGen *primary = nullptr, uint32_t max_groups = 0);
void launch_trace_resume(hipStream_t s, const SceneDev &sc, PathBuf pb, ShadowBuf sb, bool extend, bool shadow,
                         uint32_t max_items, WorkCounters *wc, const TraceSplit &split, const PrimaryGen *primary,
                         uint32_t max_groups, uint32_t *deep_stack);
inline bool resume_walk_fits(const SceneDev &sc){ return 3 * sc.wide_depth + 2 <= kResumeLdsLevels + kDeepLevels; }
size_t resume_deep_stack_words();
void launch_tri_frames(hipStream_t s, const float4 *tris, int num_tris, float4 *frames);
void launch_resolve(hipStream_t s, const Tiling &tl, PathBuf pb, float4 *accum, int samples_this_pass);
void launch_finalize(hipStream_t s, const Tiling &tl, const float4 *accum, float *d_local, float scale);
void launch_untile(hipStream_t s, const Tiling &tl, const float *d_gathered, float *d_image);

void launch_tonemap(hipStream_t s, const float *d_linear, void *d_bytes, unsigned long long num_values, int bgr, const float *d_thresholds);

void launch_probe_functions(hipStream_t s, const float *d_in, int n, float *d_out);
void launch_probe_closest(hipStream_t s, const SceneDev &sc, const float *org, const float *dir, int n, int flags,
                          float *t_out, int32_t *prim_out);
void launch_probe_visibility(hipStream_t s, const SceneDev &sc, const float *p1, const float *p2, int n, int flags,
                             int32_t *vis_out);

}
```

### path_tracing_amd/csrc/pt_kernels.hip

```cpp
#include "pt_kernels.h"
#include "pt_device_math.h"

namespace hpt {

namespace {

HPT_DEV uint32_t f2u(float f){ return __float_as_uint(f); }
HPT_DEV float u2f(uint32_t u){ return __uint_as_float(u); }
HPT_DEV f3 xyz(float4 v){ return mk3(v.x, v.y, v.z); }

HPT_DEV uint32_t bit_select(uint32_t m, uint32_t a, uint32_t b){ uint32_t r; asm("v_bfi_b32 %0, %1, %2, %3" : "=v"(r) : "v"(m), "v"(a), "v"(b)); return r; }
HPT_DEV float lo16f(uint32_t w){ float r; asm("v_cvt_f32_u32_sdwa %0, %1 dst_sel:DWORD dst_unused:UNUSED_PAD src0_sel:WORD_0" : "=v"(r) : "v"(w)); return r; }
HPT_DEV float hi16f(uint32_t w){ float r; asm("v_cvt_f32_u32_sdwa %0, %1 dst_sel:DWORD dst_unused:UNUSED_PAD src0_sel:WORD_1" : "=v"(r) : "v"(w)); return r; }

HPT_DEV uint32_t lds_push(bool want, uint32_t *lds_counter){
    unsigned long long mask = __ballot(want);
    if(mask == 0ull) return 0u;
    uint32_t lo = (uint32_t) mask, hi = (uint32_t) (mask >> 32);
    uint32_t prefix = __builtin_amdgcn_mbcnt_hi(hi, __builtin_amdgcn_mbcnt_lo(lo, 0u));
    uint32_t base = 0u;
    int leader = __ffsll((long long) mask) - 1;
    if((int) (threadIdx.x & 63u) == leader) base = atomicAdd(lds_counter, (uint32_t) __popcll(mask));
    base = (uint32_t) __shfl((int) base, leader, 64);
    return base + prefix;
// ... 548 lines not shown
                                throughput = throughput / q;
                            }
                            alive = alive && depth < max_depth;
                        }
                        if(alive){
                            HPT_SECTION(5, 2);
                            uint32_t nf = (last_is_delta ? 1u : 0u) | ((uint32_t) depth << 8) | ((uint32_t) delta_count << 16);
                            pb.org_eta[path] = make_float4(new_o.x, new_o.y, new_o.z, ray_eta);
                            pb.dir_flags[path] = make_float4(wi.x, wi.y, wi.z, u2f(nf));
                            pb.thr[path] = make_float4(throughput.x, throughput.y, throughput.z, 0.0f);
                            pb.rng[path] = make_uint2((uint32_t) rs, (uint32_t) (rs >> 32));
                        }
                    }
                }
            }
            if(PRIMARY) pb.col[path] = make_float4(first_col.x, first_col.y, first_col.z, 0.0f);
        }
        {
            const unsigned long long cm = __ballot(nee);
            if(cm != 0ull){
                const uint32_t k = (uint32_t) __popcll(cm);
                if(staged + k > 64u){ flush_nee(staged, begin); staged = 0u; }
                if(nee){
                    const uint32_t slot = staged + __builtin_amdgcn_mbcnt_hi((uint32_t) (cm >> 32), __builtin_amdgcn_mbcnt_lo((uint32_t) cm, 0u));
                    stage[0][slot] = f2u(n_wo.x); stage[1][slot] = f2u(n_wo.y); stage[2][slot] = f2u(n_wo.z);
                    stage[3][slot] = f2u(n_wi.x); stage[4][slot] = f2u(n_wi.y); stage[5][slot] = f2u(n_wi.z);
                    stage[6][slot] = f2u(n_lam); stage[7][slot] = n_mat;
                    stage[8][slot] = f2u(n_thr.x); stage[9][slot] = f2u(n_thr.y); stage[10][slot] = f2u(n_thr.z);
                    stage[11][slot] = f2u(n_pdf_light);
                    stage[12][slot] = f2u(s_p1.x); stage[13][slot] = f2u(s_p1.y); stage[14][slot] = f2u(s_p1.z);
                    stage[15][slot] = f2u(s_p2.x); stage[16][slot] = f2u(s_p2.y); stage[17][slot] = f2u(s_p2.z);
                    stage[18][slot] = path; stage[19][slot] = n_light;
                }
                staged += k;
            }
        }
        uint32_t qpos = lds_push(alive, &s_cnt[0]);
        if(alive) s_next[qpos] = path;
    }
    if(staged != 0u){ flush_nee(staged, begin); staged = 0u; }
    __syncthreads();
    if(threadIdx.x == 0){
        s_cnt[2] = s_cnt[0] ? atomicAdd(next_count, s_cnt[0]) : 0u;
        s_cnt[3] = s_cnt[1] ? atomicAdd(scount, s_cnt[1]) : 0u;
    }
    __syncthreads();
    for(uint32_t k = threadIdx.x; k < s_cnt[0]; k += kBlock) next_queue[s_cnt[2] + k] = s_next[k];
    for(uint32_t k = threadIdx.x; k < s_cnt[1]; k += kBlock) squeue[s_cnt[3] + k] = begin + k;
    if(!STRIDED) break;
    }
    if(wc){
        unsigned long long v = iters;
        for(int off = 32; off > 0; off >>= 1) v += __shfl_down(v, off, 64);
        if((threadIdx.x & 63u) == 0u && v) atomicAdd(&wc->path_iters, v);
    }
}

__global__ __launch_bounds__(kBlock)
void k_resolve(Tiling tl, PathBuf pb, float4 *accum, int samples){
    uint32_t p = blockIdx.x * kBlock + threadIdx.x;
    if(p >= (uint32_t) tl.n_local) return;
    float4 a = accum[p];
    f3 sum = mk3(a.x, a.y, a.z);
    for(int j = 0; j < samples; ++j){
        float4 c4 = pb.col[(size_t) j * tl.n_local + p];
        f3 c = xyz(c4);
        if(!is_valid_color(c)) c = mk3(0, 0, 0);
        sum = sum + c;
    }
    accum[p] = make_float4(sum.x, sum.y, sum.z, 0.0f);
}

__global__ __launch_bounds__(kBlock)
void k_tri_frames(const float4 *tris, int num_tris, float4 *frames){
    int i = blockIdx.x * kBlock + threadIdx.x;
    if(i >= num_tris) return;
    float4 t1 = tris[(size_t) i * 3 + 1], t2 = tris[(size_t) i * 3 + 2];
    f3 n = normalize3(cross3(xyz(t1), xyz(t2)));
    f3 T, B, T2, B2;
    build_local_frame(n, T, B);
    build_local_frame(n * -1.0f, T2, B2);
    frames[(size_t) i * 4 + 0] = make_float4(n.x, n.y, n.z, T.x);
    frames[(size_t) i * 4 + 1] = make_float4(T.y, T.z, B.x, B.y);
    frames[(size_t) i * 4 + 2] = make_float4(B.z, T2.x, T2.y, T2.z);
    frames[(size_t) i * 4 + 3] = make_float4(B2.x, B2.y, B2.z, t1.w);
}

__global__ __launch_bounds__(kBlock)
void k_finalize(Tiling tl, const float4 *accum, float *d_local, float divisor){
    uint32_t p = blockIdx.x * kBlock + threadIdx.x;
    if(p >= (uint32_t) tl.n_local) return;
    float4 a = accum[p];
    f3 v = mk3(a.x, a.y, a.z);
    if(divisor != 1.0f) v = v / divisor;
    d_local[(size_t) p * 3 + 0] = v.x;
    d_local[(size_t) p * 3 + 1] = v.y;
    d_local[(size_t) p * 3 + 2] = v.z;
}

__global__ __launch_bounds__(kBlock)
void k_untile(Tiling tl, const float *gathered, float *image){
    uint32_t idx = blockIdx.x * kBlock + threadIdx.x;
    if(idx >= (uint32_t) (tl.W * tl.H)) return;
    uint32_t x = idx % (uint32_t) tl.W, y = idx / (uint32_t) tl.W;
    uint32_t ts = (uint32_t) tl.tile;
    uint32_t tx = x / ts, ty = y / ts;
    uint32_t gt = ty * (uint32_t) tl.tiles_x + (tx + (uint32_t) tl.tiles_x - ty % (uint32_t) tl.tiles_x) % (uint32_t) tl.tiles_x;
    uint32_t r = gt % (uint32_t) tl.world, lt = gt / (uint32_t) tl.world;
    uint32_t bx = (x % ts) >> 3, by = (y % ts) >> 3;
    uint32_t l = ((y & 7u) << 3) | (x & 7u);
    uint32_t q = (by * (ts >> 3) + bx) * 64u + l;
    size_t src = ((size_t) r * tl.n_local + (size_t) lt * ts * ts + q) * 3;
    size_t dst = (size_t) idx * 3;
    image[dst + 0] = gathered[src + 0];
    image[dst + 1] = gathered[src + 1];
    image[dst + 2] = gathered[src + 2];
}

__global__ __launch_bounds__(kBlock)
void k_tonemap(const float *linear, uint32_t *out_words, unsigned long long num_values, int bgr, const float *thr_table){
    __shared__ float s_thr[256];
    s_thr[threadIdx.x] = thr_table[threadIdx.x];
    __syncthreads();
    unsigned long long w = (unsigned long long) blockIdx.x * kBlock + threadIdx.x;
    unsigned long long first = w * 4ull;
    if(first >= num_values) return;
    uint32_t packed = 0u;
    for(int k = 0; k < 4; ++k){
        unsigned long long j = first + (unsigned long long) k;
        if(j >= num_values) break;
        unsigned long long src = j;
        if(bgr){ unsigned long long px = j / 3ull; src = px * 3ull + (2ull - (j - px * 3ull)); }
        float x = linear[src];
        uint32_t lo = 0u;
        for(uint32_t step = 128u; step > 0u; step >>= 1) if(x >= s_thr[lo + step]) lo += step;
        packed |= lo << (8 * k);
    }
    if(first + 4ull <= num_values) out_words[w] = packed;
    else {
        unsigned char *tail = (unsigned char *) out_words + first;
        for(unsigned long long k = 0; first + k < num_values; ++k) tail[k] = (unsigned char) (packed >> (8 * k));
    }
}

#ifndef HPT_TRACE_WAVES
#define HPT_TRACE_WAVES 8
#endif
#if HPT_TRACE_WAVES > 0
#define HPT_TRACE_ATTR __attribute__((amdgpu_waves_per_eu(HPT_TRACE_WAVES, 8)))
#else
#define HPT_TRACE_ATTR
#endif
constexpr int kTraceChunk = 2048;
constexpr uint32_t kDoneCode = 0xFFFFFFFEu;
constexpr int kRefillMin = 56;
constexpr int kNodeMin = 4;
constexpr uint32_t kTraceShortQueue = 1u << 20;

template <bool ANY, bool COUNT, bool RESUME, bool TOP, bool PRIMARY>
HPT_DEV void trace_chunk(const SceneDev &sc, PathBuf pb, ShadowBuf sb, const uint32_t *queue,
                         uint32_t end, uint32_t *stk, uint32_t *s_next, int refill_min, int node_min, WorkCounters *wc,
                         uint32_t budget, DeferredRay *rec, uint32_t *s_long, uint32_t *s_nlong, const uint4 *top,
                         const PrimaryGen &pg, uint32_t *deep, uint32_t deep_stride){
    bool active = false, exhausted = false;
    uint32_t path = 0u, cur = 0u, steps = 0u;
    int sp = 0;
    f3 ro = mk3(0, 0, 0), rd = mk3(0, 0, 1);
    float ix = 0, iy = 0, iz = 0, ox = 0, oy = 0, oz = 0;
    uint32_t mx = 0u, my = 0u, mz = 0u;
    float tmax = 0.0f, limit = 0.0f, best_t = 1e20f;
    uint32_t best_prim = kHitMiss, best_ord = 0xFFFFFFFFu;
    unsigned long long n_lane_steps = 0, n_wave_steps = 0, n_boxes = 0, n_tris = 0, n_rays = 0, n_leaf_lane = 0, n_leaf_wave = 0;
    const uint32_t lane = threadIdx.x & 63u;
    const uint32_t step_limit = budget != 0u ? budget : 0xFFFFFFFFu;
    for(;;){
        if(!RESUME && budget != 0u){
            bool defer = active && steps >= budget;
            unsigned long long dm = __ballot(defer);
            if(dm != 0ull){
                uint32_t dn = (uint32_t) __popcll(dm);
                uint32_t dprefix = __builtin_amdgcn_mbcnt_hi((uint32_t) (dm >> 32), __builtin_amdgcn_mbcnt_lo((uint32_t) dm, 0u));
                int dleader = __ffsll((long long) dm) - 1;
                uint32_t dbase = 0u;
                if((int) lane == dleader) dbase = atomicAdd(s_nlong, dn);
                dbase = (uint32_t) __shfl((int) dbase, dleader, 64);
                if(defer){
                    if(!ANY && !PRIMARY && !COUNT){
                        DeferredRay *r = rec + (dbase + dprefix);
                        r->org_t = make_float4(ro.x, ro.y, ro.z, best_t);
                        r->dir_slot = make_float4(rd.x, rd.y, rd.z, u2f(path));
                        r->hit = make_uint4(best_prim, best_ord, 0u, 0u);
                    } else {
                        s_long[dbase + dprefix] = path;
                        if(!ANY) pb.hit[path] = make_uint2(f2u(best_t), best_prim);
                    }
                    active = false;
                }
            }
        }
        unsigned long long idle = __ballot(!active);
        if(idle != 0ull && !exhausted && (idle == ~0ull || __popcll(idle) >= refill_min)){
            uint32_t n = (uint32_t) __popcll(idle);
            uint32_t prefix = __builtin_amdgcn_mbcnt_hi((uint32_t) (idle >> 32), __builtin_amdgcn_mbcnt_lo((uint32_t) idle, 0u));
            int leader = __ffsll((long long) idle) - 1;
            uint32_t base = 0u;
            if((int) lane == leader) base = atomicAdd(s_next, n);
            base = (uint32_t) __shfl((int) base, leader, 64);
            exhausted = base + n >= end;
            if(!active){
                uint32_t i = base + prefix;
                if(i < end){
                    path = queue ? queue[i] : i;
                    bool start = true;
                    if(ANY){
                        float4 a = sb.org_max[path], b = sb.dir[path];
                        ro = xyz(a); rd = xyz(b); tmax = a.w;
                        if(COUNT && !RESUME) n_rays += 1;
                        for(int r = 0; r < (RESUME ? 0 : sc.num_spheres); ++r){
                            DevRound rr = sc.rounds[r];
                            float t;
                            if(hit_sphere(ro, rd, mk3(rr.c[0], rr.c[1], rr.c[2]), rr.r, tmax, t) && t > 1e-3f && (rr.flags & 1u)) start = false;
                        }
                        limit = tmax;
                    } else {
                        bool outside;
                        if(RESUME && !PRIMARY){
                            const DeferredRay *r = rec + path;
                            float4 o = r->org_t, d = r->dir_slot;
                            uint4 h = r->hit;
                            ro = xyz(o); rd = xyz(d);
                            best_t = o.w; best_prim = h.x; best_ord = h.y;
                            path = f2u(d.w);
                            limit = best_t;
                            outside = false;
                        } else if(PRIMARY){
                            uint64_t rs_unused;
                            outside = !primary_ray(pg, path, ro, rd, rs_unused);
                            if(outside && !RESUME) pb.hit[path] = make_uint2(f2u(1e20f), kHitMiss);
                        } else {
                            float4 o = pb.org_eta[path], d = pb.dir_flags[path];
                            ro = xyz(o); rd = xyz(d);
                            outside = (f2u(d.w) & 2u) != 0u;
                        }
                        if(outside) start = false;
                        else if(RESUME){
                            if(PRIMARY){
                                uint2 h = pb.hit[path];
                                best_t = u2f(h.x); best_prim = h.y; best_ord = 0xFFFFFFFFu;
                                if(best_prim != kHitMiss)
                                    best_ord = (best_prim & kHitRoundFlag) ? (best_prim & ~kHitRoundFlag) : f2u(sc.tris[(size_t) best_prim * 3].w);
                                limit = best_t;
                            }
                        } else {
                            if(COUNT) n_rays += 1;
                            best_t = 1e20f; best_prim = kHitMiss; best_ord = 0xFFFFFFFFu;
                            for(int r = 0; r < sc.num_rounds; ++r){
                                DevRound rr = sc.rounds[r];
                                float t;
                                if(hit_sphere(ro, rd, mk3(rr.c[0], rr.c[1], rr.c[2]), rr.r, 1e20f, t) && t < best_t){
                                    best_t = t; best_prim = kHitRoundFlag | (uint32_t) r; best_ord = (uint32_t) r;
                                }
                            }
                            limit = best_t;
                        }
                    }
                    if(start){
                        float dx = fabsf(rd.x) > 1e-20f ? rd.x : copysignf(1e-20f, rd.x);
                        float dy = fabsf(rd.y) > 1e-20f ? rd.y : copysignf(1e-20f, rd.y);
                        float dz = fabsf(rd.z) > 1e-20f ? rd.z : copysignf(1e-20f, rd.z);
                        if(COUNT){ ix = 1.0f / dx; iy = 1.0f / dy; iz = 1.0f / dz; }
                        else { ix = __builtin_amdgcn_rcpf(dx); iy = __builtin_amdgcn_rcpf(dy); iz = __builtin_amdgcn_rcpf(dz); }
                        ox = (sc.qorigin[0] - ro.x) * ix; oy = (sc.qorigin[1] - ro.y) * iy; oz = (sc.qorigin[2] - ro.z) * iz;
                        ix *= sc.qscale[0]; iy *= sc.qscale[1]; iz *= sc.qscale[2];
                        mx = ix < 0.0f ? 0xFFFFFFFFu : 0u; my = iy < 0.0f ? 0xFFFFFFFFu : 0u; mz = iz < 0.0f ? 0xFFFFFFFFu : 0u;
                        cur = 0u; sp = 0; steps = 0u;
                        active = true;
                    }
                }
            }
        }
        const unsigned long long idle_at_entry = __ballot(!active);
        if(idle_at_entry == ~0ull && exhausted) break;
        while(active && !(cur & kLeafFlag) && (RESUME || steps < step_limit)){
            if(node_min > 0){
                unsigned long long walking = __ballot(true);
                if(__popcll(walking) < node_min && __popcll(walking) < 64 - (int) __popcll(idle_at_entry)) break;
            }
            if(COUNT){
                n_lane_steps += 1; n_boxes += 2;
                if((int) lane == __ffsll((long long) __ballot(true)) - 1) n_wave_steps += 64;
            }
            if(!RESUME) steps += 1u;
            if(RESUME){
                const uint4 *n = sc.wnodes + (size_t) cur * 4;
                const uint4 qx = n[0], qy = n[1], qz = n[2], qc = n[3];
                const uint32_t nx01 = bit_select(mx, qx.z, qx.x), nx23 = bit_select(mx, qx.w, qx.y), fx01 = bit_select(mx, qx.x, qx.z), fx23 = bit_select(mx, qx.y, qx.w);
                const uint32_t ny01 = bit_select(my, qy.z, qy.x), ny23 = bit_select(my, qy.w, qy.y), fy01 = bit_select(my, qy.x, qy.z), fy23 = bit_select(my, qy.y, qy.w);
                const uint32_t nz01 = bit_select(mz, qz.z, qz.x), nz23 = bit_select(mz, qz.w, qz.y), fz01 = bit_select(mz, qz.x, qz.z), fz23 = bit_select(mz, qz.y, qz.w);
                const float tn0 = fmaxf(fmaxf(fmaf(lo16f(nx01), ix, ox), fmaf(lo16f(ny01), iy, oy)), fmaxf(fmaf(lo16f(nz01), iz, oz), 0.0f));
                const float tf0 = fminf(fminf(fmaf(lo16f(fx01), ix, ox), fmaf(lo16f(fy01), iy, oy)), fminf(fmaf(lo16f(fz01), iz, oz), limit));
                const float tn1 = fmaxf(fmaxf(fmaf(hi16f(nx01), ix, ox), fmaf(hi16f(ny01), iy, oy)), fmaxf(fmaf(hi16f(nz01), iz, oz), 0.0f));
                const float tf1 = fminf(fminf(fmaf(hi16f(fx01), ix, ox), fmaf(hi16f(fy01), iy, oy)), fminf(fmaf(hi16f(fz01), iz, oz), limit));
                const float tn2 = fmaxf(fmaxf(fmaf(lo16f(nx23), ix, ox), fmaf(lo16f(ny23), iy, oy)), fmaxf(fmaf(lo16f(nz23), iz, oz), 0.0f));
                const float tf2 = fminf(fminf(fmaf(lo16f(fx23), ix, ox), fmaf(lo16f(fy23), iy, oy)), fminf(fmaf(lo16f(fz23), iz, oz), limit));
                const float tn3 = fmaxf(fmaxf(fmaf(hi16f(nx23), ix, ox), fmaf(hi16f(ny23), iy, oy)), fmaxf(fmaf(hi16f(nz23), iz, oz), 0.0f));
                const float tf3 = fminf(fminf(fmaf(hi16f(fx23), ix, ox), fmaf(hi16f(fy23), iy, oy)), fminf(fmaf(hi16f(fz23), iz, oz), limit));
                const uint32_t k0 = (tn0 <= tf0 * 1.000002f && qc.x != kEmptyChild) ? (f2u(tn0) & ~3u) : 0xFFFFFFFFu;
                const uint32_t k1 = (tn1 <= tf1 * 1.000002f && qc.y != kEmptyChild) ? ((f2u(tn1) & ~3u) | 1u) : 0xFFFFFFFFu;
                const uint32_t k2 = (tn2 <= tf2 * 1.000002f && qc.z != kEmptyChild) ? ((f2u(tn2) & ~3u) | 2u) : 0xFFFFFFFFu;
                const uint32_t k3 = (tn3 <= tf3 * 1.000002f && qc.w != kEmptyChild) ? ((f2u(tn3) & ~3u) | 3u) : 0xFFFFFFFFu;
                const uint32_t kmin = min(min(k0, k1), min(k2, k3));
                const bool any = kmin != 0xFFFFFFFFu;
                const uint32_t slot = kmin & 3u;
                uint32_t near = qc.x;
                near = slot == 1u ? qc.y : near; near = slot == 2u ? qc.z : near; near = slot == 3u ? qc.w : near;
                const uint32_t c1 = ~kmin, c2 = c1 - 1u;
                const int e0 = (k0 + c1 < c2) ? 1 : 0, e1 = (k1 + c1 < c2) ? 1 : 0, e2 = (k2 + c1 < c2) ? 1 : 0, e3 = (k3 + c1 < c2) ? 1 : 0;
                uint32_t top;
                int p = sp;
                if(sp + 3 < kResumeLdsLevels){
                    top = stk[(sp > 0 ? sp - 1 : 0) * kBlock];
                    stk[(e0 ? p : kResumeLdsLevels) * kBlock] = qc.x; p += e0;
                    stk[(e1 ? p : kResumeLdsLevels) * kBlock] = qc.y; p += e1;
                    stk[(e2 ? p : kResumeLdsLevels) * kBlock] = qc.z; p += e2;
                    stk[(e3 ? p : kResumeLdsLevels) * kBlock] = qc.w; p += e3;
                } else {
                    auto level = [&](int l) -> uint32_t * { return l < kResumeLdsLevels ? stk + l * kBlock : deep + (size_t) (l - kResumeLdsLevels) * deep_stride; };
                    top = *level(sp > 0 ? sp - 1 : 0);
                    if(e0){ *level(p) = qc.x; ++p; }
                    if(e1){ *level(p) = qc.y; ++p; }
                    if(e2){ *level(p) = qc.z; ++p; }
                    if(e3){ *level(p) = qc.w; ++p; }
                }
                cur = any ? near : (sp > 0 ? top : kDoneCode);
                sp = any ? p : (sp > 0 ? sp - 1 : 0);
                continue;
            }
            const uint4 *n = TOP ? top + cur * 2u : sc.qnodes + (size_t) cur * 2;
            uint4 w0 = n[0], w1 = n[1];
            const uint32_t nx = bit_select(mx, w0.y, w0.x), fx = bit_select(mx, w0.x, w0.y);
            const uint32_t ny = bit_select(my, w0.w, w0.z), fy = bit_select(my, w0.z, w0.w);
            const uint32_t nz = bit_select(mz, w1.y, w1.x), fz = bit_select(mz, w1.x, w1.y);
            float ln = fmaxf(fmaxf(fmaf(lo16f(nx), ix, ox), fmaf(lo16f(ny), iy, oy)), fmaxf(fmaf(lo16f(nz), iz, oz), 0.0f));
            float lf = fminf(fminf(fmaf(lo16f(fx), ix, ox), fmaf(lo16f(fy), iy, oy)), fminf(fmaf(lo16f(fz), iz, oz), limit));
            float rn = fmaxf(fmaxf(fmaf(hi16f(nx), ix, ox), fmaf(hi16f(ny), iy, oy)), fmaxf(fmaf(hi16f(nz), iz, oz), 0.0f));
            float rf = fminf(fminf(fmaf(hi16f(fx), ix, ox), fmaf(hi16f(fy), iy, oy)), fminf(fmaf(hi16f(fz), iz, oz), limit));
            uint32_t lc = w1.z, rc = w1.w;
            bool hl = (ln <= lf * 1.000002f) && (lc != kEmptyChild);
            bool hr = (rn <= rf * 1.000002f) && (rc != kEmptyChild);
            bool any = hl || hr, both = hl && hr;
            bool left_first = hl && (!hr || ln <= rn);
            uint32_t top = stk[(sp > 0 ? sp - 1 : 0) * kBlock];
            stk[sp * kBlock] = left_first ? rc : lc;
            uint32_t near = left_first ? lc : rc;
            cur = any ? near : (sp > 0 ? top : kDoneCode);
            sp = any ? sp + (both ? 1 : 0) : (sp > 0 ? sp - 1 : 0);
        }
        if(active && (cur & kLeafFlag)){
            bool blocked = false, finished = cur == kDoneCode;
            if(!finished){
                if(COUNT){
                    n_leaf_lane += 1;
                    if((int) lane == __ffsll((long long) __ballot(true)) - 1) n_leaf_wave += 64;
                }
                uint32_t first = (cur & 0x7FFFFFFFu) >> 3;
                uint32_t cnt = (cur & 7u) + 1u;
                for(uint32_t k = 0; k < cnt; ++k){
                    const float4 *tp = sc.tris + (size_t) (first + k) * 3;
                    float4 t0 = tp[0], t1 = tp[1], t2 = tp[2];
                    if(COUNT) n_tris += 1;
                    float t;
                    if(hit_triangle(ro, rd, xyz(t0), xyz(t1), xyz(t2), ANY ? tmax : 1e20f, t)){
                        if(ANY){
                            if(t > 1e-3f && (f2u(t2.w) & 1u)) blocked = true;
                        } else {
                            uint32_t ord = f2u(t0.w);
                            if(t < best_t || (t == best_t && ord < best_ord)){
                                best_t = t; best_prim = first + k; best_ord = ord; limit = t;
                            }
                        }
                    }
                }
                if(ANY && blocked) finished = true;
                else if(sp > 0){
                    --sp;
                    cur = (RESUME && sp >= kResumeLdsLevels) ? deep[(size_t) (sp - kResumeLdsLevels) * deep_stride] : stk[sp * kBlock];
                }
                else finished = true;
            }
            if(finished){
                active = false;
                if(!ANY) pb.hit[path] = make_uint2(f2u(best_t), best_prim);
                else if(!blocked){
                    float4 c = sb.contrib[path];
                    const uint32_t slot = f2u(c.w);
                    float4 col = pb.col[slot];
                    col.x = col.x + c.x; col.y = col.y + c.y; col.z = col.z + c.z;
                    pb.col[slot] = col;
                }
            }
        }
    }
    if(COUNT){
        for(int off = 32; off > 0; off >>= 1){
            n_boxes += __shfl_down(n_boxes, off, 64); n_tris += __shfl_down(n_tris, off, 64);
            n_rays += __shfl_down(n_rays, off, 64); n_lane_steps += __shfl_down(n_lane_steps, off, 64);
            n_wave_steps += __shfl_down(n_wave_steps, off, 64); n_leaf_lane += __shfl_down(n_leaf_lane, off, 64);
            n_leaf_wave += __shfl_down(n_leaf_wave, off, 64);
        }
        if(lane == 0u){
            if(n_boxes) atomicAdd(ANY ? &wc->boxes_shadow : &wc->boxes_closest, n_boxes);
            if(n_tris) atomicAdd(ANY ? &wc->tris_shadow : &wc->tris_closest, n_tris);
            if(n_rays) atomicAdd(ANY ? &wc->shadow_rays : &wc->closest_rays, n_rays);
            if(n_lane_steps) atomicAdd(ANY ? &wc->lane_steps_shadow : &wc->lane_steps_closest, n_lane_steps);
            if(n_wave_steps) atomicAdd(ANY ? &wc->wave_steps_shadow : &wc->wave_steps_closest, n_wave_steps);
            if(n_leaf_lane) atomicAdd(ANY ? &wc->leaf_lane_shadow : &wc->leaf_lane_closest, n_leaf_lane);
            if(n_leaf_wave) atomicAdd(ANY ? &wc->leaf_wave_shadow : &wc->leaf_wave_closest, n_leaf_wave);
        }
    }
}

struct LongQueues { uint32_t *equeue, *ecount, *squeue, *scount; uint32_t budget; DeferredRay *rec; };

template <bool COUNT, bool RESUME, bool TOP, bool PRIMARY>
__global__ __launch_bounds__(kBlock) HPT_TRACE_ATTR
void k_trace(SceneDev sc, PathBuf pb, ShadowBuf sb, const uint32_t *equeue, const uint32_t *ecount_ptr,
             const uint32_t *squeue, const uint32_t *scount_ptr, uint32_t chunk_rays, int refill_min, int node_min,
             int stack_words, LongQueues lq, WorkCounters *wc, PrimaryGen pg, uint32_t *deep){
    extern __shared__ uint32_t s_dyn_stack[];
    __shared__ uint32_t s_next, s_nlong, s_gbase;
    __shared__ uint4 s_top[TOP ? kTopNodes * 2 : 1];
    uint32_t *s_long = s_dyn_stack + stack_words;
    if(TOP){
        const uint32_t words = (uint32_t) (sc.num_nodes < kTopNodes ? sc.num_nodes : kTopNodes) * 2u;
        for(uint32_t i = threadIdx.x; i < words; i += kBlock) s_top[i] = sc.qnodes[i];
    }
    uint32_t ecount = ecount_ptr ? *ecount_ptr : 0u, scount = scount_ptr ? *scount_ptr : 0u;
    uint32_t ce = ecount >= kTraceShortQueue ? chunk_rays : (uint32_t) kBlock;
    uint32_t cs = scount >= kTraceShortQueue ? chunk_rays : (uint32_t) kBlock;
    uint32_t ne = (ecount + ce - 1) / ce, ns = (scount + cs - 1) / cs;
    for(uint32_t bid = blockIdx.x; bid < ne + ns; bid += gridDim.x){
        bool shadow = bid >= ne;
        uint32_t chunk = shadow ? bid - ne : bid;
        uint32_t csize = shadow ? cs : ce;
        uint32_t begin = chunk * csize;
        uint32_t total = shadow ? scount : ecount;
        uint32_t end = begin + csize < total ? begin + csize : total;
        const bool records = !shadow && !PRIMARY && !COUNT;
        const uint32_t lbase = records ? begin : 0u;
        if(threadIdx.x == 0){ s_next = begin; s_nlong = lbase; }
        __syncthreads();
        uint32_t *deep_lane = RESUME ? deep + (size_t) blockIdx.x * kBlock + threadIdx.x : nullptr;
        const uint32_t deep_stride = gridDim.x * kBlock;
        if(shadow) trace_chunk<true, COUNT, RESUME, TOP, false>(sc, pb, sb, squeue, end, s_dyn_stack + threadIdx.x, &s_next, refill_min, node_min, wc,
                                                                lq.budget, lq.rec, s_long, &s_nlong, s_top, pg, deep_lane, deep_stride);
        else trace_chunk<false, COUNT, RESUME, TOP, PRIMARY>(sc, pb, sb, equeue, end, s_dyn_stack + threadIdx.x, &s_next, refill_min, node_min, wc,
                                                             lq.budget, lq.rec, s_long, &s_nlong, s_top, pg, deep_lane, deep_stride);
        __syncthreads();
        if(!RESUME && lq.budget != 0u){
            uint32_t n = s_nlong - lbase;
            if(n != 0u){
                if(threadIdx.x == 0) s_gbase = atomicAdd(shadow ? lq.scount : lq.ecount, n);
                __syncthreads();
                uint32_t *dst = (shadow ? lq.squeue : lq.equeue) + s_gbase;
                for(uint32_t i = threadIdx.x; i < n; i += kBlock) dst[i] = records ? begin + i : s_long[i];
            }
        }
        __syncthreads();
    }
}

template <bool BRUTE>
__global__ __launch_bounds__(kBlock)
void k_probe_closest(SceneDev sc, const float *org, const float *dir, int n, float *t_out, int32_t *prim_out){
    __shared__ uint32_t s_stack[kStackDepth * kBlock];
    int i = blockIdx.x * kBlock + threadIdx.x;
    if(i >= n) return;
    Tally tally; tally.boxes = 0; tally.tris = 0; tally.steps = 0; tally.wave_steps = 0;
    float t; uint32_t prim;
    closest_hit<BRUTE, false>(sc, mk3(org[3 * i], org[3 * i + 1], org[3 * i + 2]), mk3(dir[3 * i], dir[3 * i + 1], dir[3 * i + 2]),
                              s_stack + threadIdx.x, t, prim, tally);
    int32_t ord = -1;
    if(prim != kHitMiss){
        if(prim & kHitRoundFlag) ord = (int32_t) (prim & 0x7FFFFFFFu);
        else ord = (int32_t) f2u(sc.tris[(size_t) prim * 3].w);
    }
    t_out[i] = t; prim_out[i] = ord;
}

template <bool BRUTE>
__global__ __launch_bounds__(kBlock)
void k_probe_visibility(SceneDev sc, const float *p1, const float *p2, int n, int32_t *vis_out){
    __shared__ uint32_t s_stack[kStackDepth * kBlock];
    int i = blockIdx.x * kBlock + threadIdx.x;
    if(i >= n) return;
    Tally tally; tally.boxes = 0; tally.tris = 0; tally.steps = 0; tally.wave_steps = 0;
    f3 a = mk3(p1[3 * i], p1[3 * i + 1], p1[3 * i + 2]), b = mk3(p2[3 * i], p2[3 * i + 1], p2[3 * i + 2]);
    f3 diff = b - a;
    float dist = length3(diff);
    f3 d = diff / dist;
    vis_out[i] = segment_visible<BRUTE, false>(sc, a, d, dist - 1e-3f, s_stack + threadIdx.x, tally) ? 1 : 0;
}

__global__ __launch_bounds__(kBlock)
void k_probe_functions(const float *in, int n, float *out){
    int i = blockIdx.x * kBlock + threadIdx.x;
    if(i >= n) return;
    const float *r = in + (size_t) i * 24;
    float *o = out + (size_t) i * 40;
    Mat m; m.base = mk3(r[0], r[1], r[2]); m.roughness = r[3]; m.metallic = r[4]; m.eta = r[5];
    f3 N = mk3(r[6], r[7], r[8]), wo_w = mk3(r[9], r[10], r[11]), wi_w = mk3(r[12], r[13], r[14]);
    ShadeCtx ctx = make_shade_ctx(N, wo_w);
    ShadePre pre;
    pre.diffuse = m.base / kPi * (1.0f - m.metallic);
    const float alpha = roughness_to_alpha(m.roughness);
    pre.lam_o = ggx_lambda(ctx.wo, alpha);
    f3 f; float pdf;
    bsdf_eval_pdf(m, ctx, wi_w, f, pdf, &pre);
    o[0] = f.x; o[1] = f.y; o[2] = f.z; o[3] = pdf;
    f3 swi, sf; float spdf, new_eta; bool is_delta;
    bsdf_sample(m, ctx, r[15], r[16], r[17], r[18], swi, sf, spdf, is_delta, new_eta, &pre);
    o[4] = swi.x; o[5] = swi.y; o[6] = swi.z; o[7] = sf.x; o[8] = sf.y; o[9] = sf.z; o[10] = spdf;
    o[11] = is_delta ? 1.0f : 0.0f; o[12] = new_eta;
    o[13] = fr_dielectric(r[19], r[20], r[21]);
    f3 sch = fr_schlick(r[19], m.base);
    o[14] = sch.x; o[15] = sch.y; o[16] = sch.z;
    f3 wi_l = to_local(wi_w, ctx.T, ctx.B, ctx.N);
    o[17] = ggx_D(wi_l, alpha); o[18] = ggx_lambda(wi_l, alpha); o[19] = ggx_G(ctx.wo, wi_l, alpha);
    float sn, cs; sincos_2pi(r[17], sn, cs);
    o[20] = sn; o[21] = cs;
    f3 vn = sample_visible_normal(ctx.wo.z > 0 ? ctx.wo : ctx.wo * -1.0f, alpha, sqrtf(r[16]), sn, cs);
    o[22] = vn.x; o[23] = vn.y; o[24] = vn.z;
    o[25] = is_valid_color(f) ? 1.0f : 0.0f;
    f3 cl = clamp_radiance(f * 20.0f, 15.0f);
    o[26] = cl.x; o[27] = cl.y; o[28] = cl.z;
    o[29] = ctx.T.x; o[30] = ctx.T.y; o[31] = ctx.T.z; o[32] = ctx.B.x; o[33] = ctx.B.y; o[34] = ctx.B.z;
    o[35] = ctx.wo.x; o[36] = ctx.wo.y; o[37] = ctx.wo.z;
    o[38] = 0.0f; o[39] = 0.0f;
}

uint32_t grid_for(uint32_t items){
    uint32_t g = (items + kBlock - 1) / kBlock;
    if(g < 1u) g = 1u;
    return g > 2048u ? 2048u : g;
}

}


void launch_generate(hipStream_t s, const Tiling &tl, const CameraDev &cam, PathBuf pb,
                     uint32_t *qcount, int samples_this_pass, uint32_t first_sample, uint64_t seed,
                     WorkCounters *wc){
    uint32_t total = (uint32_t) tl.n_local * (uint32_t) samples_this_pass;
    hipLaunchKernelGGL(k_generate, dim3(grid_for(total)), dim3(kBlock), 0, s, tl, cam, pb, qcount, total,
                       first_sample, seed, wc);
}

void launch_extend(hipStream_t s, const SceneDev &sc, PathBuf pb, const uint32_t *queue, const uint32_t *qcount,
                   uint32_t max_items, int flags, WorkCounters *wc){
    dim3 g(grid_for(max_items)), b(kBlock);
    bool brute = flags & 1, count = flags & 2;
    if(brute && count) hipLaunchKernelGGL((k_extend<true, true>), g, b, 0, s, sc, pb, queue, qcount, wc);
    else if(brute) hipLaunchKernelGGL((k_extend<true, false>), g, b, 0, s, sc, pb, queue, qcount, wc);
    else if(count) hipLaunchKernelGGL((k_extend<false, true>), g, b, 0, s, sc, pb, queue, qcount, wc);
    else hipLaunchKernelGGL((k_extend<false, false>), g, b, 0, s, sc, pb, queue, qcount, wc);
}

void launch_shade(hipStream_t s, const SceneDev &sc, PathBuf pb, const uint32_t *queue, const uint32_t *qcount,
                  uint32_t max_items, uint32_t *next_queue, uint32_t *next_count, ShadowBuf sb, uint32_t *squeue,
                  uint32_t *scount, int max_depth, int max_delta, int roulette, WorkCounters *wc, const PrimaryGen *primary,
                  uint32_t max_groups){
    uint32_t g = (max_items + kShadeChunk - 1) / kShadeChunk;
    if(g < (uint32_t) kShadeTargetGroups) g = (uint32_t) kShadeTargetGroups;
    uint32_t small = (max_items + kBlock - 1) / kBlock;
    if(small < g) g = small < 1u ? 1u : small;
    const bool strided = max_groups != 0u && g > max_groups;
    if(strided) g = max_groups;
    PrimaryGen none{};
    if(primary) hipLaunchKernelGGL((k_shade<true, false>), dim3(g), dim3(kBlock), 0, s, sc, pb, queue, qcount, next_queue,
                                   next_count, sb, squeue, scount, max_depth, max_delta, roulette, wc, *primary);
    else if(strided) hipLaunchKernelGGL((k_shade<false, true>), dim3(g), dim3(kBlock), 0, s, sc, pb, queue, qcount, next_queue,
                                        next_count, sb, squeue, scount, max_depth, max_delta, roulette, wc, none);
    else hipLaunchKernelGGL((k_shade<false, false>), dim3(g), dim3(kBlock), 0, s, sc, pb, queue, qcount, next_queue,
                            next_count, sb, squeue, scount, max_depth, max_delta, roulette, wc, none);
}

void launch_connect(hipStream_t s, const SceneDev &sc, PathBuf pb, ShadowBuf sb, const uint32_t *squeue,
                    const uint32_t *scount, uint32_t max_items, int flags, WorkCounters *wc){
// ... 117 lines not shown
```

### path_tracing_amd/csrc/scene_build.cpp

```cpp
#include "hpt_scene.h"

#include <algorithm>
#include <chrono>
#include <cmath>
#include <cstddef>
#include <cstdio>
#include <cstdlib>
#include <cstring>
#include <map>
#include <array>
#include <atomic>
#include <condition_variable>
#include <deque>
#include <functional>
#include <memory>
#include <mutex>
#include <thread>
#ifdef __linux__
#include <sched.h>
#endif

namespace hpt {
namespace {

// ... 408 lines not shown
}

void pack_wide_boxes(HostScene &hs){
    parallel_chunks(hs.wnodes.size(), [&](int, size_t b0, size_t e0){
        for(size_t qi = b0; qi < e0; ++qi){
            WideNode &w = hs.wnodes[qi];
            uint32_t lo[3][4], hi[3][4];
            for(int k = 0; k < 4; ++k){
                const uint32_t src = hs.wide_src[qi * 4 + (size_t) k];
                if(src != kEmptyChild){
                    const BvhNode &b = hs.nodes[src >> 1];
                    const float *mn = (src & 1u) ? b.rmin : b.lmin, *mx = (src & 1u) ? b.rmax : b.lmax;
                    for(int a = 0; a < 3; ++a){ lo[a][k] = grid_lo(mn[a], hs.qorigin[a], hs.qscale[a]); hi[a][k] = grid_hi(mx[a], hs.qorigin[a], hs.qscale[a]); }
                }
                else { for(int a = 0; a < 3; ++a){ lo[a][k] = 65535u; hi[a][k] = 0u; } }
            }
            for(int a = 0; a < 3; ++a){
                w.w[a * 4 + 0] = lo[a][0] | (lo[a][1] << 16); w.w[a * 4 + 1] = lo[a][2] | (lo[a][3] << 16);
                w.w[a * 4 + 2] = hi[a][0] | (hi[a][1] << 16); w.w[a * 4 + 3] = hi[a][2] | (hi[a][3] << 16);
            }
        }
    });
}

}

void grid_of_box(const float lo_in[3], const float hi_in[3], float qorigin[3], float qscale[3]){
    for(int a = 0; a < 3; ++a){
        float lo = lo_in[a], hi = hi_in[a];
        if(!(lo <= hi)){ lo = 0.0f; hi = 1.0f; }
        qorigin[a] = lo;
        float ext = hi - lo;
        qscale[a] = ext > 0.0f ? ext / 65535.0f : 1.0f;
        qscale[a] = std::nextafter(qscale[a], INFINITY);
    }
}

float box_padding_of(const float scene_min[3], const float scene_max[3], int nt){
    Box b; for(int a = 0; a < 3; ++a){ b.mn[a] = scene_min[a]; b.mx[a] = scene_max[a]; }
    return box_padding(b, nt);
}

const char *flatten_rounds_host(const void *lights_v, int nl, const void *spheres_v, int ns, const uint32_t *sphere_material,
                                std::vector<DevRound> &rounds, std::vector<DevLight> &lights_out){
    if(nl < 0 || ns < 0) return "negative primitive count";
    if((nl > 0 && !lights_v) || (ns > 0 && (!spheres_v || !sphere_material))) return "null primitive array";
    const RefLight *lights = (const RefLight *) lights_v;
    const RefSphere *spheres = (const RefSphere *) spheres_v;
    rounds.clear(); rounds.reserve((size_t) ns + nl);
    for(int i = 0; i < ns; ++i){
        DevRound r; memset(&r, 0, sizeof r);
        r.c[0] = spheres[i].c[0]; r.c[1] = spheres[i].c[1]; r.c[2] = spheres[i].c[2]; r.r = spheres[i].r;
        r.material = sphere_material[i];
        r.flags = (spheres[i].m.eta <= 0.0f) ? 1u : 0u;
        rounds.push_back(r);
    }
    for(int i = 0; i < nl; ++i){
        DevRound r; memset(&r, 0, sizeof r);
        const RefSphere &b = lights[i].ball;
        r.c[0] = b.c[0]; r.c[1] = b.c[1]; r.c[2] = b.c[2]; r.r = b.r;
        r.material = (uint32_t) i;
        r.flags = 2u;
        rounds.push_back(r);
    }
    lights_out.clear(); lights_out.reserve(nl);
    for(int i = 0; i < nl; ++i){
        const RefLight &L = lights[i];
        DevLight d; memset(&d, 0, sizeof d);
        d.raw_dir[0] = L.dir[0]; d.raw_dir[1] = L.dir[1]; d.raw_dir[2] = L.dir[2];
        d.ball_c[0] = L.ball.c[0]; d.ball_c[1] = L.ball.c[1]; d.ball_c[2] = L.ball.c[2];
        d.pos[0] = L.pos[0]; d.pos[1] = L.pos[1]; d.pos[2] = L.pos[2];
        d.r = L.ball.r;
        normalize3(L.dir, 1.0f, d.main_dir);
        normalize3(L.dir, -1.0f, d.neg_dir);
        d.cos_cutoff = cosf(L.cutoff);
        d.cutoff = L.cutoff;
        d.illum[0] = L.illum[0]; d.illum[1] = L.illum[1]; d.illum[2] = L.illum[2];
        d.area = 4.0f * kPi * L.ball.r * L.ball.r;
        d.is_parallel = L.is_parallel ? 1u : 0u;
        d.cone_ratio = (1.0f - d.cos_cutoff) / 2.0f;
        lights_out.push_back(d);
    }
    return "";
}

const char *check_triangle_update(const void *kept_v, int kept_nt, const void *tris_v, int nt, char *msg, size_t msg_cap){
    if(nt < 0) return "negative triangle count";
    if(nt != kept_nt){ snprintf(msg, msg_cap, "an update keeps the triangle count: the scene has %d triangles, %d were handed over", kept_nt, nt); return msg; }
    if(nt > 0 && !tris_v) return "null triangle array";
    const RefTriangle *kept = (const RefTriangle *) kept_v, *tris = (const RefTriangle *) tris_v;
    for(int i = 0; i < nt; ++i)
        if(memcmp(&kept[i].o, &tris[i].o, sizeof(RefTriangle) - offsetof(RefTriangle, o)) != 0){
            snprintf(msg, msg_cap, "an update moves vertices only: material or id bytes of triangle %d differ from the record the scene was created from", i);
            return msg;
        }
    return "";
}

const char *check_rounds_update(const void *kept_spheres_v, int kept_ns, int kept_nl, const void *lights_v, int nl, const void *spheres_v, int ns,
                                char *msg, size_t msg_cap){
    if(nl < 0 || ns < 0) return "negative primitive count";
    if(nl != kept_nl || ns != kept_ns){ snprintf(msg, msg_cap, "an update keeps the counts: the scene has %d lights and %d spheres, %d and %d were handed over", kept_nl, kept_ns, nl, ns); return msg; }
    if((nl > 0 && !lights_v) || (ns > 0 && !spheres_v)) return "null primitive array";
    const RefSphere *kept = (const RefSphere *) kept_spheres_v, *spheres = (const RefSphere *) spheres_v;
    for(int i = 0; i < ns; ++i)
        if(memcmp(&kept[i].o, &spheres[i].o, sizeof(RefSphere) - offsetof(RefSphere, o)) != 0){
            snprintf(msg, msg_cap, "an update moves spheres only: material or id bytes of sphere %d differ from the record the scene was created from", i);
            return msg;
        }
    return "";
}

const char *refit_host_scene(HostScene &hs, const void *tris_v, int nt, uint64_t *dead_out){
    if(nt != hs.num_tris) return "an update keeps the triangle count";
    if(nt > 0 && !tris_v) return "null triangle array";
    if(hs.level_begin.size() < 2 || hs.wide_src.size() != hs.wnodes.size() * 4) return "internal error: the scene keeps no refit tables";
    const RefTriangle *tris = (const RefTriangle *) tris_v;
    const uint32_t num_rounds = (uint32_t) (hs.num_spheres + hs.num_lights);
    pod_vector<Box> tb((size_t) nt);
    Box scene_box;
    const size_t ndead = triangle_boxes(tris, nt, scene_box, [&](size_t i, const Box &b, bool){ tb[i] = b; });
    if(dead_out) *dead_out = ndead;
    const float pad_abs = box_padding(scene_box, nt);
    parallel_chunks((size_t) nt, [&](int, size_t b0, size_t e0){
        for(size_t s = b0; s < e0; ++s) triangle_geometry(hs.tris[s], tris[hs.tris[s].ordinal - num_rounds]);
    });
    pod_vector<Box> exact(hs.nodes.size());
    for(size_t l = hs.level_begin.size() - 1; l-- > 0; ){
        const size_t first = hs.level_begin[l], cnt = hs.level_begin[l + 1] - first;
        parallel_chunks(cnt, [&](int, size_t b0, size_t e0){
            for(size_t i = first + b0; i < first + e0; ++i){
                BvhNode &n = hs.nodes[i];
                Box both; both.reset();
                for(int side = 0; side < 2; ++side){
                    const uint32_t code = side ? n.right : n.left;
                    float *mn = side ? n.rmin : n.lmin, *mx = side ? n.rmax : n.lmax;
                    if(code == kEmptyChild){ set_empty_box(mn, mx); continue; }
                    Box cb;
                    if(code & kLeafFlag){
                        cb.reset();
                        const uint32_t s0 = (code & ~kLeafFlag) >> 3, c = (code & 7u) + 1u;
                        for(uint32_t s = s0; s < s0 + c; ++s) cb.grow(tb[hs.tris[s].ordinal - num_rounds]);
                    } else cb = exact[code];
                    write_padded_box(mn, mx, cb, pad_abs);
                    both.grow(cb);
                }
                exact[i] = both;
            }
        });
    }
    quantise_tree(hs);
    pack_wide_boxes(hs);
    return "";
}

const char *build_host_scene(const void *lights_v, int nl, const void *spheres_v, int ns,
                             const void *tris_v, int nt, HostScene &hs){
    if(nl < 0 || ns < 0 || nt < 0) return "negative primitive count";
    if((nl > 0 && !lights_v) || (ns > 0 && !spheres_v) || (nt > 0 && !tris_v)) return "null primitive array";
    if((uint64_t) nt >= (1ull << 28)) return "too many triangles (limit 2^28)";
    const RefSphere *spheres = (const RefSphere *) spheres_v;
    const RefTriangle *tris = (const RefTriangle *) tris_v;

    hs = HostScene();
    hs.num_spheres = ns; hs.num_lights = nl; hs.num_tris = nt;
    std::map<MatKey, uint32_t> mat_table;

    {
        std::vector<uint32_t> sphere_material((size_t) ns);
        for(int i = 0; i < ns; ++i) sphere_material[(size_t) i] = intern_material(spheres[i].m, mat_table, hs.materials);
        const char *e = flatten_rounds_host(lights_v, nl, spheres_v, ns, sphere_material.data(), hs.rounds, hs.lights);
        if(e && *e) return e;
    }

    auto t0 = std::chrono::steady_clock::now();
#ifdef HPT_DEV_TUNING
    auto tp = t0;
    auto lap = [&](const char *what){ auto n = std::chrono::steady_clock::now(); fprintf(stderr, "  build phase %-12s %.1f ms\n", what, std::chrono::duration<double, std::milli>(n - tp).count()); tp = n; };
#else
    auto lap = [](const char *){};
#endif
    Builder B;
#ifdef HPT_DEV_TUNING
    if(const char *e = getenv("HPT_MAX_LEAF")){ int v = atoi(e); if(v >= 1 && v <= 8) B.max_leaf = v; }
#endif
    B.prims.resize(nt);
    Box scene_box;
    triangle_boxes(tris, nt, scene_box, [&](size_t i, const Box &b, bool live){
        Prim &p = B.prims[i];
        p.index = (uint32_t) i;
        p.box = b;
        for(int a = 0; a < 3; ++a) p.cen[a] = live ? 0.5f * (b.mn[a] + b.mx[a]) : b.mn[a];
    });
    B.pad_abs = box_padding(scene_box, nt);
    B.nodes.resize((nt > 0 ? (size_t) nt : 1) + Builder::kSlotSlack);
    lap("prims");

    if(nt == 0){
        BvhNode n; memset(&n, 0, sizeof n);
        set_empty_box(n.lmin, n.lmax); set_empty_box(n.rmin, n.rmax);
        n.left = n.right = kEmptyChild;
        B.nodes[0] = n; B.next_node = 1;
    } else if(nt <= B.max_leaf){
        BvhNode n; memset(&n, 0, sizeof n);
        B.nodes[0] = n; B.next_node = 1;
        Box lb;
        uint32_t lc = B.build(0, nt, 1, lb);
        B.write_box(B.nodes[0].lmin, B.nodes[0].lmax, lb); B.nodes[0].left = lc;
        set_empty_box(B.nodes[0].rmin, B.nodes[0].rmax); B.nodes[0].right = kEmptyChild;
    } else {
        Box rb;
        uint32_t root = B.build(0, nt, 0, rb);
        if(root != 0) return "internal error: BVH root is not node 0";
    }
    lap("tree");
    B.nodes.resize(B.next_node.load());
    hs.nodes.swap(B.nodes);
    hs.bvh_depth = B.max_depth_seen.load();
    {
        const size_t n = hs.nodes.size();
        pod_vector<uint32_t> order(n);
        pod_vector<uint32_t> new_index(n);
        auto inner = [](uint32_t c){ return c != kEmptyChild && !(c & kLeafFlag); };
        size_t lvl_begin = 0, lvl_end = 1;
        order[0] = 0u;
        while(lvl_begin < lvl_end){
            hs.level_begin.push_back((uint32_t) lvl_begin);
            const size_t cnt = lvl_end - lvl_begin;
            size_t per_chunk[kChunks] = {};
            parallel_chunks(cnt, [&](int c, size_t b0, size_t e0){
                size_t k = 0;
                for(size_t i = b0; i < e0; ++i){ const BvhNode &nd = hs.nodes[order[lvl_begin + i]]; k += (inner(nd.left) ? 1u : 0u) + (inner(nd.right) ? 1u : 0u); }
                per_chunk[c] = k;
            });
            size_t offs[kChunks], total = 0;
            for(int c = 0; c < kChunks; ++c){ offs[c] = total; total += per_chunk[c]; }
            if(lvl_end + total > n) return "internal error: BVH has more reachable nodes than slots";
            parallel_chunks(cnt, [&](int c, size_t b0, size_t e0){
                size_t o = lvl_end + offs[c];
                for(size_t i = b0; i < e0; ++i){
                    const BvhNode &nd = hs.nodes[order[lvl_begin + i]];
                    if(inner(nd.left)){ new_index[nd.left] = (uint32_t) o; order[o++] = nd.left; }
                    if(inner(nd.right)){ new_index[nd.right] = (uint32_t) o; order[o++] = nd.right; }
                }
            });
            lvl_begin = lvl_end; lvl_end += total;
        }
        hs.level_begin.push_back((uint32_t) lvl_end);
        order.resize(lvl_end);
        const size_t reachable = order.size();
        pod_vector<BvhNode> sorted(reachable);
        parallel_chunks(reachable, [&](int, size_t b0, size_t e0){
            for(size_t i = b0; i < e0; ++i){
                BvhNode nd = hs.nodes[order[i]];
                if(nd.left != kEmptyChild && !(nd.left & kLeafFlag)) nd.left = new_index[nd.left];
                if(nd.right != kEmptyChild && !(nd.right & kLeafFlag)) nd.right = new_index[nd.right];
                sorted[i] = nd;
            }
        });
        hs.nodes.swap(sorted);
    }
    lap("renumber");
    quantise_tree(hs);
    if(hs.bvh_depth > kMaxBvhDepth) return "internal error: BVH deeper than the traversal stack";
    lap("quantise");
    {
        struct Kid { const float *mn, *mx; uint32_t code, src; };
        auto half_area = [](const Kid &k){ float dx = k.mx[0] - k.mn[0], dy = k.mx[1] - k.mn[1], dz = k.mx[2] - k.mn[2]; return dx * dy + dy * dz + dz * dx; };
        struct Kids { Kid k[4]; int n; uint32_t code[4]; };
        pod_vector<uint32_t> todo(hs.nodes.size() + 1);
        pod_vector<Kids> all(hs.nodes.size() + 1);
        todo[0] = 0u;
        size_t lvl_begin = 0, lvl_end = 1;
        while(lvl_begin < lvl_end){
            const size_t cnt = lvl_end - lvl_begin;
            size_t per_chunk[kChunks] = {};
            parallel_chunks(cnt, [&](int c, size_t b0, size_t e0){
                size_t inner_kids = 0;
                for(size_t i = b0; i < e0; ++i){
                    Kids ks; ks.n = 0;
                    auto open = [&](uint32_t idx){
                        const BvhNode &b = hs.nodes[idx];
                        if(b.left != kEmptyChild) ks.k[ks.n++] = Kid{ b.lmin, b.lmax, b.left, idx * 2u };
                        if(b.right != kEmptyChild) ks.k[ks.n++] = Kid{ b.rmin, b.rmax, b.right, idx * 2u + 1u };
                    };
                    open(todo[lvl_begin + i]);
                    while(ks.n < 4){
                        int best = -1; float ba = -1.0f;
                        for(int k = 0; k < ks.n; ++k) if(!(ks.k[k].code & kLeafFlag)){ float a = half_area(ks.k[k]); if(a > ba){ ba = a; best = k; } }
                        if(best < 0) break;
                        uint32_t cc = ks.k[best].code;
                        ks.k[best] = ks.k[ks.n - 1]; --ks.n;
                        open(cc);
                    }
                    for(int k = 0; k < ks.n; ++k) if(!(ks.k[k].code & kLeafFlag)) ++inner_kids;
                    all[lvl_begin + i] = ks;
                }
                per_chunk[c] = inner_kids;
            });
            size_t offs[kChunks], total = 0;
            for(int c = 0; c < kChunks; ++c){ offs[c] = total; total += per_chunk[c]; }
            parallel_chunks(cnt, [&](int c, size_t b0, size_t e0){
                size_t o = lvl_end + offs[c];
                for(size_t i = b0; i < e0; ++i){
                    Kids &ks = all[lvl_begin + i];
                    for(int k = 0; k < 4; ++k){
                        if(k >= ks.n) ks.code[k] = kEmptyChild;
                        else if(ks.k[k].code & kLeafFlag) ks.code[k] = ks.k[k].code;
                        else { ks.code[k] = (uint32_t) o; todo[o++] = ks.k[k].code; }
                    }
                }
            });
            ++hs.wide_depth;
            lvl_begin = lvl_end; lvl_end += total;
        }
        all.resize(lvl_end);
        hs.wnodes.resize(all.size());
        hs.wide_src.resize(all.size() * 4);
        parallel_chunks(all.size(), [&](int, size_t b0, size_t e0){
            for(size_t qi = b0; qi < e0; ++qi){
                const Kids &ks = all[qi];
                for(int k = 0; k < 4; ++k){
                    hs.wnodes[qi].w[12 + k] = ks.code[k];
                    hs.wide_src[qi * 4 + (size_t) k] = k < ks.n ? ks.k[k].src : kEmptyChild;
                }
            }
        });
        pack_wide_boxes(hs);
    }

    lap("wide");
    hs.tris.resize(nt);
    pod_vector<uint32_t> mat_of((size_t) nt);
    {   RefMat last; memset(&last, 0xFF, sizeof last); uint32_t last_idx = 0; bool have = false;
        for(int i = 0; i < nt; ++i){
            const RefMat &m = tris[i].m;
            if(!have || memcmp(&m, &last, 28) != 0){ last_idx = intern_material(m, mat_table, hs.materials); last = m; have = true; }
            mat_of[(size_t) i] = last_idx;
        }
    }
    parallel_chunks((size_t) nt, [&](int, size_t b0, size_t e0){
        for(size_t s = b0; s < e0; ++s){
            const RefTriangle &t = tris[B.prims[s].index];
            DevTriangle &d = hs.tris[s];
            triangle_geometry(d, t);
            d.ordinal = (uint32_t) (ns + nl) + B.prims[s].index;
            d.material = mat_of[B.prims[s].index];
            d.flags = (t.m.eta <= 0.0f) ? 1u : 0u;
        }
    });
    lap("triangles");
    auto t1 = std::chrono::steady_clock::now();
    hs.ms_bvh_build = std::chrono::duration<double, std::milli>(t1 - t0).count();
    if(hs.materials.empty()){ DevMaterial m; memset(&m, 0, sizeof m); hs.materials.push_back(m); }
    return "";
}


const char *build_bdpt_host_scene(const void *lights_v, int nl, const void *spheres_v, int ns, const void *tris_v, int nt,
                                  const int32_t *obj_kind, const int32_t *obj_index, const int32_t *obj_group, int nobj,
                                  HostBdptScene &out){
    if(nl < 0 || ns < 0 || nt < 0) return "negative primitive count";
    if((nl > 0 && !lights_v) || (ns > 0 && !spheres_v) || (nt > 0 && !tris_v)) return "null primitive array";
    const RefSphere *spheres = (const RefSphere *) spheres_v;
    const RefTriangle *tris = (const RefTriangle *) tris_v;
    out = HostBdptScene();
    {
        HostScene tmp;
        const char *e = build_host_scene(lights_v, nl, nullptr, 0, nullptr, 0, tmp);
        if(e && *e) return e;
        out.lights = tmp.lights;
    }
    struct Item { int kind, index; uint32_t seq; };
    std::map<int, std::vector<Item>> gm;
    uint32_t seq = 0;
    if(obj_kind && obj_index && obj_group){
        for(int i = 0; i < nobj; ++i){
            if(obj_kind[i] == 0 ? (obj_index[i] < 0 || obj_index[i] >= ns) : (obj_index[i] < 0 || obj_index[i] >= nt)) return "object index out of range";
            gm[obj_group[i]].push_back(Item{ obj_kind[i], obj_index[i], 0u });
        }
    } else {
        for(int i = 0; i < ns; ++i) gm[0].push_back(Item{ 0, i, 0u });
        for(int i = 0; i < nt; ++i) gm[0].push_back(Item{ 1, i, 0u });
    }
    for(auto &kv : gm) for(Item &it : kv.second) it.seq = seq++;

    std::map<MatKey, uint32_t> mat_table;
    Box scene_box; scene_box.reset();
    std::vector<Box> gboxes;
    for(auto &kv : gm){
        Box gb; for(int a = 0; a < 3; ++a){ gb.mn[a] = 99999.f; gb.mx[a] = -99999.f; }
        for(const Item &it : kv.second){
            if(it.kind == 0){
                const RefSphere &s = spheres[it.index];
                for(int a = 0; a < 3; ++a){
                    gb.mn[a] = std::min({ gb.mn[a], s.c[a] + s.r, s.c[a] - s.r });
                    gb.mx[a] = std::max({ gb.mx[a], s.c[a] + s.r, s.c[a] - s.r });
                }
            } else {
                const RefTriangle &t = tris[it.index];
                const float *vv[3] = { t.v0, t.v1, t.v2 };
                for(int k = 0; k < 3; ++k) for(int a = 0; a < 3; ++a){ gb.mn[a] = std::min(gb.mn[a], vv[k][a]); gb.mx[a] = std::max(gb.mx[a], vv[k][a]); }
            }
        }
        for(int a = 0; a < 3; ++a) for(int guard = 0; guard < 64 && gb.mx[a] - gb.mn[a] < 1e-6f; ++guard){ gb.mn[a] -= 0.5f * 1e-6f; gb.mx[a] += 0.5f * 1e-6f; }
        gboxes.push_back(gb);
        scene_box.grow(gb);
    }
    for(int a = 0; a < 3; ++a){ out.scene_min[a] = 1e9f; out.scene_max[a] = -1e9f; }
    for(const Box &gb : gboxes) for(int a = 0; a < 3; ++a){ out.scene_min[a] = std::min(out.scene_min[a], gb.mn[a]); out.scene_max[a] = std::max(out.scene_max[a], gb.mx[a]); }
    float extent = 0.0f;
    if(!gboxes.empty()) for(int a = 0; a < 3; ++a){
        extent = std::max(extent, scene_box.mx[a] - scene_box.mn[a]);
        extent = std::max(extent, std::max(std::fabs(scene_box.mn[a]), std::fabs(scene_box.mx[a])));
    }
    size_t gi = 0;
    for(auto &kv : gm){
        DevGroup g; memset(&g, 0, sizeof g);
        for(int a = 0; a < 3; ++a){ g.mn[a] = gboxes[gi].mn[a]; g.mx[a] = gboxes[gi].mx[a]; }
        g.sphere_first = (uint32_t) out.spheres.size();
        std::vector<Item> gtris;
        for(const Item &it : kv.second){
            if(it.kind == 0){
                const RefSphere &s = spheres[it.index];
                DevRound r; memset(&r, 0, sizeof r);
                r.c[0] = s.c[0]; r.c[1] = s.c[1]; r.c[2] = s.c[2]; r.r = s.r;
                r.material = intern_material(s.m, mat_table, out.materials);
                r.flags = (s.m.eta <= 0.0f) ? 1u : 0u;
                r.pad[0] = it.seq;
                out.spheres.push_back(r);
            } else gtris.push_back(it);
        }
        g.sphere_count = (uint32_t) out.spheres.size() - g.sphere_first;
        Builder B;
        B.node_base = (uint32_t) out.nodes.size(); B.tri_base = (uint32_t) out.tris.size();
        B.pad_abs = 2e-6f * extent;
        B.prims.resize(gtris.size());
        for(size_t i = 0; i < gtris.size(); ++i){
            const RefTriangle &t = tris[gtris[i].index];
            Prim &p = B.prims[i];
            p.box.reset(); p.box.grow(t.v0); p.box.grow(t.v1); p.box.grow(t.v2);
            for(int a = 0; a < 3; ++a) p.cen[a] = 0.5f * (p.box.mn[a] + p.box.mx[a]);
            p.index = (uint32_t) i;
        }
        B.nodes.resize(std::max<size_t>(gtris.size(), 1) + Builder::kSlotSlack);
        if(gtris.empty()) g.root = kEmptyChild;
        else { Box rb; g.root = B.build(0, (int) gtris.size(), 0, rb); }
        if(B.max_depth_seen.load() > kMaxBvhDepth) return "internal error: BVH deeper than the traversal stack";
        out.bvh_depth = std::max(out.bvh_depth, B.max_depth_seen.load());
        out.nodes.insert(out.nodes.end(), B.nodes.begin(), B.nodes.begin() + B.next_node.load());
        for(const Prim &pr : B.prims){
            const Item &it = gtris[pr.index];
            const RefTriangle &t = tris[it.index];
            DevTriangle d;
            for(int a = 0; a < 3; ++a){ d.v0[a] = t.v0[a]; d.e1[a] = t.v1[a] - t.v0[a]; d.e2[a] = t.v2[a] - t.v0[a]; }
            d.ordinal = it.seq;
            d.material = intern_material(t.m, mat_table, out.materials);
            d.flags = (t.m.eta <= 0.0f) ? 1u : 0u;
            out.tris.push_back(d);
        }
        out.groups.push_back(g);
        ++gi;
    }
    if(out.materials.empty()){ DevMaterial m; memset(&m, 0, sizeof m); out.materials.push_back(m); }
    if(out.nodes.empty()){ BvhNode n; memset(&n, 0, sizeof n); out.nodes.push_back(n); }
    return "";
}

}
```

Measured before the change: 2510 Msamples/s.

## Start BVH traversal from a shared-memory root treelet of up to eight children

Builds a small root treelet on the host by repeatedly opening the largest-area inner nodes near the BVH root into up to kRootWide children. The treelet is uploaded and staged in LDS per block. Each ray tests all treelet boxes at setup, starts at the nearest hit child and keeps a bitmask of the other hits to resume from when a subtree finishes. This skips the top few binary levels and their stack pushes for every ray, at the cost of extra LDS, registers and per-ray box tests. It also replaces the separate `limit` variable with a macro over tmax/best_t.

```diff
diff --git a/include/hpt.h b/include/hpt.h
--- a/include/hpt.h
+++ b/include/hpt.h
@@ -266,6 +266,12 @@
 int hpt_scene_export_bvh(const hpt_scene *scene, hpt_bvh_info *info,
                          void *qnodes_out, size_t qnodes_cap, void *tris_out, size_t tris_cap);
 
+int hpt_bvh_export_root_treelet_host(const void *lights, int num_lights, const void *spheres, int num_spheres,
+                                     const void *triangles, const void *new_triangles, int num_triangles,
+                                     uint32_t *binary_out, int32_t *num_binary, uint32_t *wide_out, int32_t *num_wide,
+                                     void *wnodes_out, size_t wnodes_cap, int32_t *num_wnodes);
+int hpt_root_treelet_width(void);
+
 int hpt_trace_closest(hpt_scene *scene, const float *origins, const float *dirs, int n,
                       int flags, float *t_out, int32_t *prim_out);
 int hpt_trace_visibility(hpt_scene *scene, const float *p1, const float *p2, int n,
diff --git a/path_tracing_amd/__init__.py b/path_tracing_amd/__init__.py
--- a/path_tracing_amd/__init__.py
+++ b/path_tracing_amd/__init__.py
@@ -155,7 +155,7 @@
                      "hpt_denoiser_run_guided", "hpt_denoiser_estimate_variance", "hpt_history_length", "hpt_guided_check",
                      "hpt_history_create_flags", "hpt_history_variance", "hpt_history_read_moments", "hpt_history_variance_check",
                      "hpt_scene_update_triangles", "hpt_scene_update_rounds", "hpt_scene_update_check", "hpt_scene_get_update_info",
-                     "hpt_bvh_refit_host"):
+                     "hpt_bvh_refit_host", "hpt_bvh_export_root_treelet_host", "hpt_root_treelet_width"):
             if hasattr(lib, name):
                 getattr(lib, name).restype = C.c_int
         if hasattr(lib, "hpt_sppm_destroy"):
@@ -715,6 +715,35 @@
         _vp(lights), len(lights), _vp(spheres), len(spheres), _vp(triangles), _vp(new_triangles), len(triangles), info, qn, qcap, tr, tcap))
 
 
+def root_treelet_width() -> int:
+    return int(load_library().hpt_root_treelet_width())
+
+
+def export_root_treelet_host(lights, spheres, triangles, new_triangles=None) -> dict:
+    lib = load_library()
+    lights = np.ascontiguousarray(lights, LIGHT)
+    spheres = np.ascontiguousarray(spheres, SPHERE)
+    triangles = np.ascontiguousarray(triangles, TRIANGLE)
+    new = None
+    if new_triangles is not None:
+        new = np.ascontiguousarray(new_triangles, TRIANGLE)
+        if len(new) != len(triangles):
+            raise HptError("hpt error 1: an update keeps the triangle count: %d triangles, %d were handed over" % (len(triangles), len(new)))
+    width = root_treelet_width()
+    b = np.zeros((width, 4), np.uint32); w = np.zeros((width, 4), np.uint32)
+    nb = C.c_int32(); nw = C.c_int32(); nn = C.c_int32()
+
+    def call(wn, cap):
+        _check(lib.hpt_bvh_export_root_treelet_host(
+            _vp(lights), len(lights), _vp(spheres), len(spheres), _vp(triangles), _vp(new) if new is not None else None, len(triangles),
+            b.ctypes.data_as(C.POINTER(C.c_uint32)), C.byref(nb), w.ctypes.data_as(C.POINTER(C.c_uint32)), C.byref(nw),
+            wn, C.c_size_t(cap), C.byref(nn)))
+    call(None, 0)
+    wn = np.zeros((max(nn.value, 1), 16), np.uint32)
+    call(_vp(wn), wn.nbytes)
+    return {"width": width, "binary": b[:nb.value].copy(), "wide": w[:nw.value].copy(), "wnodes": wn[:nn.value]}
+
+
 def update_check(scene, triangles, num_triangles=None) -> None:
     tr = np.ascontiguousarray(triangles, TRIANGLE) if triangles is not None else None
     n = len(tr) if num_triangles is None else int(num_triangles)
diff --git a/path_tracing_amd/csrc/hpt_api.cpp b/path_tracing_amd/csrc/hpt_api.cpp
--- a/path_tracing_amd/csrc/hpt_api.cpp
+++ b/path_tracing_amd/csrc/hpt_api.cpp
@@ -219,6 +219,19 @@
     if(e == hipSuccess) e = s->geo.nodes.upload(hs.nodes);
     if(e == hipSuccess) e = s->geo.qnodes.upload(hs.qnodes);
     if(e == hipSuccess) e = s->geo.wnodes.upload(hs.wnodes);
+    if(e == hipSuccess){
+        std::vector<RootChild> rt((size_t) 2 * kRootWide + 1, RootChild{ 0u, 0u, kEmptyChild, 0u });
+        const std::vector<RootChild> *lists[2] = { &hs.root_binary, &hs.root_wide };
+        for(int w = 0; w < 2; ++w){
+            RootChild *d = rt.data() + (size_t) w * kRootWide;
+            if(lists[w]->empty()) d[0] = RootChild{ kEmptyChild, 0u, 0u, 0u };
+            for(size_t k = 0; k < lists[w]->size() && k < (size_t) kRootWide; ++k) d[k] = (*lists[w])[k];
+        }
+        uint32_t deepest = 0u;
+        for(const RootChild &c : hs.root_binary) deepest = std::max(deepest, c.depth);
+        rt.back() = RootChild{ deepest, 0u, 0u, 0u };
+        e = s->geo.root_treelet.upload(rt);
+    }
     if(e == hipSuccess) e = s->geo.tris.upload(hs.tris);
     if(e == hipSuccess) e = s->geo.rounds.upload(hs.rounds);
     if(e == hipSuccess) e = s->geo.mats.upload(hs.materials);
@@ -235,6 +248,7 @@
     s->geo.sd.tri_frames = s->geo.tri_frames.get();
     s->geo.sd.qnodes = (const uint4 *) s->geo.qnodes.get();
     s->geo.sd.wnodes = (const uint4 *) s->geo.wnodes.get(); s->geo.sd.wide_depth = hs.wide_depth;
+    s->geo.sd.root_treelet = (const uint4 *) s->geo.root_treelet.get();
     for(int a = 0; a < 3; ++a){ s->geo.sd.qorigin[a] = hs.qorigin[a]; s->geo.sd.qscale[a] = hs.qscale[a]; }
     s->geo.sd.rounds = s->geo.rounds.get(); s->geo.sd.mats = s->geo.mats.get(); s->geo.sd.lights = s->geo.lights.get();
     s->geo.sd.num_rounds = ns + nl; s->geo.sd.num_spheres = ns; s->geo.sd.num_lights = nl; s->geo.sd.num_tris = nt;
@@ -515,6 +529,33 @@
     return export_host_tree(hs, info, qnodes_out, qnodes_cap, tris_out, tris_cap);
 }
 
+int hpt_bvh_export_root_treelet_host(const void *lights, int nl, const void *spheres, int ns, const void *tris, const void *new_tris, int nt,
+                                     uint32_t *binary_out, int32_t *num_binary, uint32_t *wide_out, int32_t *num_wide,
+                                     void *wnodes_out, size_t wnodes_cap, int32_t *num_wnodes){
+    if(!num_binary || !num_wide) return fail(HPT_ERR_INVALID, "null count");
+    HostScene hs;
+    const char *err = build_host_scene(lights, nl, spheres, ns, tris, nt, hs);
+    if(err && *err) return fail(HPT_ERR_INVALID, err);
+    if(new_tris){
+        char msg[200];
+        err = check_triangle_update(tris, nt, new_tris, nt, msg, sizeof msg);
+        if(err && *err) return fail(HPT_ERR_INVALID, err);
+        err = refit_host_scene(hs, new_tris, nt);
+        if(err && *err) return fail(HPT_ERR_INVALID, err);
+    }
+    *num_binary = (int32_t) hs.root_binary.size(); *num_wide = (int32_t) hs.root_wide.size();
+    if(binary_out && !hs.root_binary.empty()) memcpy(binary_out, hs.root_binary.data(), hs.root_binary.size() * sizeof(RootChild));
+    if(wide_out && !hs.root_wide.empty()) memcpy(wide_out, hs.root_wide.data(), hs.root_wide.size() * sizeof(RootChild));
+    if(num_wnodes) *num_wnodes = (int32_t) hs.wnodes.size();
+    if(wnodes_out){
+        if(wnodes_cap < hs.wnodes.size() * sizeof(WideNode)) return fail(HPT_ERR_INVALID, "wnodes_out too small");
+        memcpy(wnodes_out, hs.wnodes.data(), hs.wnodes.size() * sizeof(WideNode));
+    }
+    return HPT_OK;
+}
+
+int hpt_root_treelet_width(void){ return kRootWide; }
+
 int hpt_scene_export_bvh(const hpt_scene *s, hpt_bvh_info *info, void *qnodes_out, size_t qnodes_cap, void *tris_out, size_t tris_cap){
     if(!s || !info) return fail(HPT_ERR_INVALID, "null argument");
     if(int rcd = on_scene_device(s)) return rcd;
diff --git a/path_tracing_amd/csrc/hpt_host.h b/path_tracing_amd/csrc/hpt_host.h
--- a/path_tracing_amd/csrc/hpt_host.h
+++ b/path_tracing_amd/csrc/hpt_host.h
@@ -73,6 +73,7 @@
     struct Geometry {
         hpt::SceneDev sd{};
         hpt::DevBuf<hpt::BvhNode> nodes; hpt::DevBuf<hpt::QBvhNode> qnodes; hpt::DevBuf<hpt::WideNode> wnodes;
+        hpt::DevBuf<hpt::RootChild> root_treelet;
         hpt::DevBuf<hpt::DevTriangle> tris; hpt::DevBuf<hpt::DevRound> rounds;
         hpt::DevBuf<hpt::DevMaterial> mats; hpt::DevBuf<hpt::DevLight> lights;
         hpt::DevBuf<float4> tri_frames;
diff --git a/path_tracing_amd/csrc/hpt_scene.h b/path_tracing_amd/csrc/hpt_scene.h
--- a/path_tracing_amd/csrc/hpt_scene.h
+++ b/path_tracing_amd/csrc/hpt_scene.h
@@ -11,6 +11,11 @@
 constexpr int kMaxLeafTris = 2;
 constexpr int kMaxBvhDepth = 30;
 constexpr int kStackDepth = 32;
+#ifndef HPT_ROOT_WIDE
+#define HPT_ROOT_WIDE 8
+#endif
+constexpr int kRootWide = HPT_ROOT_WIDE;
+static_assert(kRootWide >= 2 && kRootWide <= 8 && kRootWide % 2 == 0, "root treelet width");
 
 struct Float4 { float x, y, z, w; };
 
@@ -37,6 +42,8 @@
 };
 
 struct WideNode { uint32_t w[16]; };
+
+struct RootChild { uint32_t src, slot, code, depth; };
 
 struct DevTriangle {
     float v0[3]; uint32_t ordinal;
@@ -70,6 +77,7 @@
 
 static_assert(sizeof(BvhNode) == 64 && sizeof(DevTriangle) == 48 && sizeof(DevRound) == 32, "layout");
 static_assert(sizeof(QBvhNode) == 32 && sizeof(WideNode) == 64, "layout");
+static_assert(sizeof(RootChild) == 16, "layout");
 static_assert(sizeof(DevMaterial) == 48 && sizeof(DevLight) == 112, "layout");
 
 struct HostScene {
@@ -79,6 +87,7 @@
     int wide_depth = 0;
     pod_vector<uint32_t> wide_src;
     std::vector<uint32_t> level_begin;
+    std::vector<RootChild> root_binary, root_wide;
     float qorigin[3] = {0, 0, 0}, qscale[3] = {1, 1, 1};
     pod_vector<DevTriangle> tris;
     std::vector<DevRound> rounds;
diff --git a/path_tracing_amd/csrc/pt_kernels.h b/path_tracing_amd/csrc/pt_kernels.h
--- a/path_tracing_amd/csrc/pt_kernels.h
+++ b/path_tracing_amd/csrc/pt_kernels.h
@@ -10,6 +10,7 @@
     const uint4 *qnodes;
     const uint4 *wnodes;
     int wide_depth;
+    const uint4 *root_treelet;
     float qorigin[3], qscale[3];
     const float4 *tris;
     const float4 *tri_frames;
diff --git a/path_tracing_amd/csrc/pt_kernels.hip b/path_tracing_amd/csrc/pt_kernels.hip
--- a/path_tracing_amd/csrc/pt_kernels.hip
+++ b/path_tracing_amd/csrc/pt_kernels.hip
@@ -724,8 +724,16 @@
 #define HPT_TRACE_ATTR
 #endif
 constexpr int kTraceChunk = 2048;
+constexpr int kTreeletVec = kRootWide + (kRootWide + 4) / 4;
 constexpr uint32_t kDoneCode = 0xFFFFFFFEu;
-constexpr int kRefillMin = 56;
+#ifndef HPT_REFILL_MIN
+#define HPT_REFILL_MIN 56
+#endif
+#ifndef HPT_ROOT_RESUME
+#define HPT_ROOT_RESUME 0
+#endif
+constexpr bool kRootResume = HPT_ROOT_RESUME != 0;
+constexpr int kRefillMin = HPT_REFILL_MIN;
 constexpr int kNodeMin = 4;
 constexpr uint32_t kTraceShortQueue = 1u << 20;
 
@@ -736,11 +744,14 @@
                          const PrimaryGen &pg, uint32_t *deep, uint32_t deep_stride){
     bool active = false, exhausted = false;
     uint32_t path = 0u, cur = 0u, steps = 0u;
+    uint32_t pending = 0u;
+    const uint32_t *tw = (const uint32_t *) top;
     int sp = 0;
     f3 ro = mk3(0, 0, 0), rd = mk3(0, 0, 1);
     float ix = 0, iy = 0, iz = 0, ox = 0, oy = 0, oz = 0;
     uint32_t mx = 0u, my = 0u, mz = 0u;
-    float tmax = 0.0f, limit = 0.0f, best_t = 1e20f;
+#define HPT_LIMIT (ANY ? tmax : best_t)
+    float tmax = 0.0f, best_t = 1e20f;
     uint32_t best_prim = kHitMiss, best_ord = 0xFFFFFFFFu;
     unsigned long long n_lane_steps = 0, n_wave_steps = 0, n_boxes = 0, n_tris = 0, n_rays = 0, n_leaf_lane = 0, n_leaf_wave = 0;
     const uint32_t lane = threadIdx.x & 63u;
@@ -793,7 +804,6 @@
                             float t;
                             if(hit_sphere(ro, rd, mk3(rr.c[0], rr.c[1], rr.c[2]), rr.r, tmax, t) && t > 1e-3f && (rr.flags & 1u)) start = false;
                         }
-                        limit = tmax;
                     } else {
                         bool outside;
                         if(RESUME && !PRIMARY){
@@ -803,7 +813,6 @@
                             ro = xyz(o); rd = xyz(d);
                             best_t = o.w; best_prim = h.x; best_ord = h.y;
                             path = f2u(d.w);
-                            limit = best_t;
                             outside = false;
                         } else if(PRIMARY){
                             uint64_t rs_unused;
@@ -821,7 +830,6 @@
                                 best_t = u2f(h.x); best_prim = h.y; best_ord = 0xFFFFFFFFu;
                                 if(best_prim != kHitMiss)
                                     best_ord = (best_prim & kHitRoundFlag) ? (best_prim & ~kHitRoundFlag) : f2u(sc.tris[(size_t) best_prim * 3].w);
-                                limit = best_t;
                             }
                         } else {
                             if(COUNT) n_rays += 1;
@@ -833,7 +841,6 @@
                                     best_t = t; best_prim = kHitRoundFlag | (uint32_t) r; best_ord = (uint32_t) r;
                                 }
                             }
-                            limit = best_t;
                         }
                     }
                     if(start){
@@ -845,7 +852,34 @@
                         ox = (sc.qorigin[0] - ro.x) * ix; oy = (sc.qorigin[1] - ro.y) * iy; oz = (sc.qorigin[2] - ro.z) * iz;
                         ix *= sc.qscale[0]; iy *= sc.qscale[1]; iz *= sc.qscale[2];
                         mx = ix < 0.0f ? 0xFFFFFFFFu : 0u; my = iy < 0.0f ? 0xFFFFFFFFu : 0u; mz = iz < 0.0f ? 0xFFFFFFFFu : 0u;
-                        cur = 0u; sp = 0; steps = 0u;
+                        sp = 0; steps = 0u;
+                        if(COUNT || (RESUME && !kRootResume)) cur = 0u;
+                        else {
+                            uint32_t kmin = 0xFFFFFFFFu, hits = 0u;
+#pragma unroll
+                            for(int p = kRootWide / 2 - 1; p >= 0; --p){
+                                const uint4 w0 = top[2 * p], w1 = top[2 * p + 1];
+                                const uint32_t nx = bit_select(mx, w0.y, w0.x), fx = bit_select(mx, w0.x, w0.y);
+                                const uint32_t ny = bit_select(my, w0.w, w0.z), fy = bit_select(my, w0.z, w0.w);
+                                const uint32_t nz = bit_select(mz, w1.y, w1.x), fz = bit_select(mz, w1.x, w1.y);
+                                const float ln = fmaxf(fmaxf(fmaf(lo16f(nx), ix, ox), fmaf(lo16f(ny), iy, oy)), fmaxf(fmaf(lo16f(nz), iz, oz), 0.0f));
+                                const float lf = fminf(fminf(fmaf(lo16f(fx), ix, ox), fmaf(lo16f(fy), iy, oy)), fminf(fmaf(lo16f(fz), iz, oz), HPT_LIMIT));
+                                const float rn = fmaxf(fmaxf(fmaf(hi16f(nx), ix, ox), fmaf(hi16f(ny), iy, oy)), fmaxf(fmaf(hi16f(nz), iz, oz), 0.0f));
+                                const float rf = fminf(fminf(fmaf(hi16f(fx), ix, ox), fmaf(hi16f(fy), iy, oy)), fminf(fmaf(hi16f(fz), iz, oz), HPT_LIMIT));
+                                const bool hl = (ln <= lf * 1.000002f) && (w1.z != kEmptyChild);
+                                const bool hr = (rn <= rf * 1.000002f) && (w1.w != kEmptyChild);
+                                const uint32_t kl = hl ? ((f2u(ln) & ~7u) | (uint32_t) (2 * p)) : 0xFFFFFFFFu;
+                                const uint32_t kr = hr ? ((f2u(rn) & ~7u) | (uint32_t) (2 * p + 1)) : 0xFFFFFFFFu;
+                                kmin = min(kmin, min(kl, kr));
+                                hits = (hits << 2) | (hl ? 1u : 0u) | (hr ? 2u : 0u);
+                                asm volatile("" ::: "memory");
+                            }
+                            const bool any = kmin != 0xFFFFFFFFu;
+                            const uint32_t slot = kmin & 7u;
+                            cur = any ? tw[(slot >> 1) * 8u + 6u + (slot & 1u)] : kDoneCode;
+                            pending = hits & ~(1u << slot);
+                            if(!RESUME) steps = tw[kRootWide * 4 + (any ? slot : (uint32_t) kRootWide)];
+                        }
                         active = true;
                     }
                 }
@@ -870,13 +904,13 @@
                 const uint32_t ny01 = bit_select(my, qy.z, qy.x), ny23 = bit_select(my, qy.w, qy.y), fy01 = bit_select(my, qy.x, qy.z), fy23 = bit_select(my, qy.y, qy.w);
                 const uint32_t nz01 = bit_select(mz, qz.z, qz.x), nz23 = bit_select(mz, qz.w, qz.y), fz01 = bit_select(mz, qz.x, qz.z), fz23 = bit_select(mz, qz.y, qz.w);
                 const float tn0 = fmaxf(fmaxf(fmaf(lo16f(nx01), ix, ox), fmaf(lo16f(ny01), iy, oy)), fmaxf(fmaf(lo16f(nz01), iz, oz), 0.0f));
-                const float tf0 = fminf(fminf(fmaf(lo16f(fx01), ix, ox), fmaf(lo16f(fy01), iy, oy)), fminf(fmaf(lo16f(fz01), iz, oz), limit));
+                const float tf0 = fminf(fminf(fmaf(lo16f(fx01), ix, ox), fmaf(lo16f(fy01), iy, oy)), fminf(fmaf(lo16f(fz01), iz, oz), HPT_LIMIT));
                 const float tn1 = fmaxf(fmaxf(fmaf(hi16f(nx01), ix, ox), fmaf(hi16f(ny01), iy, oy)), fmaxf(fmaf(hi16f(nz01), iz, oz), 0.0f));
-                const float tf1 = fminf(fminf(fmaf(hi16f(fx01), ix, ox), fmaf(hi16f(fy01), iy, oy)), fminf(fmaf(hi16f(fz01), iz, oz), limit));
+                const float tf1 = fminf(fminf(fmaf(hi16f(fx01), ix, ox), fmaf(hi16f(fy01), iy, oy)), fminf(fmaf(hi16f(fz01), iz, oz), HPT_LIMIT));
                 const float tn2 = fmaxf(fmaxf(fmaf(lo16f(nx23), ix, ox), fmaf(lo16f(ny23), iy, oy)), fmaxf(fmaf(lo16f(nz23), iz, oz), 0.0f));
-                const float tf2 = fminf(fminf(fmaf(lo16f(fx23), ix, ox), fmaf(lo16f(fy23), iy, oy)), fminf(fmaf(lo16f(fz23), iz, oz), limit));
+                const float tf2 = fminf(fminf(fmaf(lo16f(fx23), ix, ox), fmaf(lo16f(fy23), iy, oy)), fminf(fmaf(lo16f(fz23), iz, oz), HPT_LIMIT));
                 const float tn3 = fmaxf(fmaxf(fmaf(hi16f(nx23), ix, ox), fmaf(hi16f(ny23), iy, oy)), fmaxf(fmaf(hi16f(nz23), iz, oz), 0.0f));
-                const float tf3 = fminf(fminf(fmaf(hi16f(fx23), ix, ox), fmaf(hi16f(fy23), iy, oy)), fminf(fmaf(hi16f(fz23), iz, oz), limit));
+                const float tf3 = fminf(fminf(fmaf(hi16f(fx23), ix, ox), fmaf(hi16f(fy23), iy, oy)), fminf(fmaf(hi16f(fz23), iz, oz), HPT_LIMIT));
                 const uint32_t k0 = (tn0 <= tf0 * 1.000002f && qc.x != kEmptyChild) ? (f2u(tn0) & ~3u) : 0xFFFFFFFFu;
                 const uint32_t k1 = (tn1 <= tf1 * 1.000002f && qc.y != kEmptyChild) ? ((f2u(tn1) & ~3u) | 1u) : 0xFFFFFFFFu;
                 const uint32_t k2 = (tn2 <= tf2 * 1.000002f && qc.z != kEmptyChild) ? ((f2u(tn2) & ~3u) | 2u) : 0xFFFFFFFFu;
@@ -908,15 +942,15 @@
                 sp = any ? p : (sp > 0 ? sp - 1 : 0);
                 continue;
             }
-            const uint4 *n = TOP ? top + cur * 2u : sc.qnodes + (size_t) cur * 2;
+            const uint4 *n = TOP ? top + kTreeletVec + cur * 2u : sc.qnodes + (size_t) cur * 2;
             uint4 w0 = n[0], w1 = n[1];
             const uint32_t nx = bit_select(mx, w0.y, w0.x), fx = bit_select(mx, w0.x, w0.y);
             const uint32_t ny = bit_select(my, w0.w, w0.z), fy = bit_select(my, w0.z, w0.w);
             const uint32_t nz = bit_select(mz, w1.y, w1.x), fz = bit_select(mz, w1.x, w1.y);
             float ln = fmaxf(fmaxf(fmaf(lo16f(nx), ix, ox), fmaf(lo16f(ny), iy, oy)), fmaxf(fmaf(lo16f(nz), iz, oz), 0.0f));
-            float lf = fminf(fminf(fmaf(lo16f(fx), ix, ox), fmaf(lo16f(fy), iy, oy)), fminf(fmaf(lo16f(fz), iz, oz), limit));
+            float lf = fminf(fminf(fmaf(lo16f(fx), ix, ox), fmaf(lo16f(fy), iy, oy)), fminf(fmaf(lo16f(fz), iz, oz), HPT_LIMIT));
             float rn = fmaxf(fmaxf(fmaf(hi16f(nx), ix, ox), fmaf(hi16f(ny), iy, oy)), fmaxf(fmaf(hi16f(nz), iz, oz), 0.0f));
-            float rf = fminf(fminf(fmaf(hi16f(fx), ix, ox), fmaf(hi16f(fy), iy, oy)), fminf(fmaf(hi16f(fz), iz, oz), limit));
+            float rf = fminf(fminf(fmaf(hi16f(fx), ix, ox), fmaf(hi16f(fy), iy, oy)), fminf(fmaf(hi16f(fz), iz, oz), HPT_LIMIT));
             uint32_t lc = w1.z, rc = w1.w;
             bool hl = (ln <= lf * 1.000002f) && (lc != kEmptyChild);
             bool hr = (rn <= rf * 1.000002f) && (rc != kEmptyChild);
@@ -928,7 +962,7 @@
             cur = any ? near : (sp > 0 ? top : kDoneCode);
             sp = any ? sp + (both ? 1 : 0) : (sp > 0 ? sp - 1 : 0);
         }
-        if(active && (cur & kLeafFlag)){
+        if(active && (cur & kLeafFlag) && (RESUME || COUNT || steps <= step_limit)){
             bool blocked = false, finished = cur == kDoneCode;
             if(!finished){
                 if(COUNT){
@@ -948,7 +982,7 @@
                         } else {
                             uint32_t ord = f2u(t0.w);
                             if(t < best_t || (t == best_t && ord < best_ord)){
-                                best_t = t; best_prim = first + k; best_ord = ord; limit = t;
+                                best_t = t; best_prim = first + k; best_ord = ord;
                             }
                         }
                     }
@@ -960,6 +994,31 @@
                 }
                 else finished = true;
             }
+            if(!COUNT && finished && pending != 0u && !(ANY && blocked)){
+                do {
+                    const uint32_t k = (uint32_t) __ffs((int) pending) - 1u;
+                    pending &= pending - 1u;
+                    const uint32_t *w = tw + (k >> 1) * 8u;
+                    bool hit = true;
+                    if(!ANY){
+                        const uint32_t sh = (k & 1u) * 16u;
+                        const uint32_t x0 = w[0] >> sh, x1 = w[1] >> sh;
+                        float tn = fmaxf(fmaf(lo16f(bit_select(mx, x1, x0)), ix, ox), 0.0f), tf = fminf(fmaf(lo16f(bit_select(mx, x0, x1)), ix, ox), HPT_LIMIT);
+                        asm volatile("" ::: "memory");
+                        const uint32_t y0 = w[2] >> sh, y1 = w[3] >> sh;
+                        tn = fmaxf(tn, fmaf(lo16f(bit_select(my, y1, y0)), iy, oy)); tf = fminf(tf, fmaf(lo16f(bit_select(my, y0, y1)), iy, oy));
+                        asm volatile("" ::: "memory");
+                        const uint32_t z0 = w[4] >> sh, z1 = w[5] >> sh;
+                        tn = fmaxf(tn, fmaf(lo16f(bit_select(mz, z1, z0)), iz, oz)); tf = fminf(tf, fmaf(lo16f(bit_select(mz, z0, z1)), iz, oz));
+                        hit = tn <= tf * 1.000002f;
+                    }
+                    if(hit){
+                        cur = w[6u + (k & 1u)];
+                        if(!RESUME) steps = max(steps, tw[kRootWide * 4 + k]);
+                        finished = false;
+                    }
+                } while(finished && pending != 0u);
+            }
             if(finished){
                 active = false;
                 if(!ANY) pb.hit[path] = make_uint2(f2u(best_t), best_prim);
@@ -992,6 +1051,8 @@
     }
 }
 
+#undef HPT_LIMIT
+
 struct LongQueues { uint32_t *equeue, *ecount, *squeue, *scount; uint32_t budget; DeferredRay *rec; };
 
 template <bool COUNT, bool RESUME, bool TOP, bool PRIMARY>
@@ -1001,11 +1062,41 @@
              int stack_words, LongQueues lq, WorkCounters *wc, PrimaryGen pg, uint32_t *deep){
     extern __shared__ uint32_t s_dyn_stack[];
     __shared__ uint32_t s_next, s_nlong, s_gbase;
-    __shared__ uint4 s_top[TOP ? kTopNodes * 2 : 1];
+    __shared__ uint4 s_top[kTreeletVec + (TOP ? kTopNodes * 2 : 0)];
     uint32_t *s_long = s_dyn_stack + stack_words;
     if(TOP){
         const uint32_t words = (uint32_t) (sc.num_nodes < kTopNodes ? sc.num_nodes : kTopNodes) * 2u;
-        for(uint32_t i = threadIdx.x; i < words; i += kBlock) s_top[i] = sc.qnodes[i];
+        for(uint32_t i = threadIdx.x; i < words; i += kBlock) s_top[kTreeletVec + i] = sc.qnodes[i];
+    }
+    if(!COUNT && (!RESUME || kRootResume) && threadIdx.x < (uint32_t) (kRootWide / 2)){
+        uint32_t lo[2][3], hi[2][3], code[2], start[2];
+        for(int c = 0; c < 2; ++c){
+            const uint4 d = sc.root_treelet[(RESUME ? kRootWide : 0) + 2 * (int) threadIdx.x + c];
+            code[c] = d.z; start[c] = RESUME ? 0u : d.w;
+            for(int a = 0; a < 3; ++a){ lo[c][a] = 65535u; hi[c][a] = 0u; }
+            if(d.z == kEmptyChild) continue;
+            if(d.x == kEmptyChild){
+                for(int a = 0; a < 3; ++a){ lo[c][a] = 0u; hi[c][a] = 65535u; }
+                continue;
+            }
+            const uint32_t sh = (d.y & 1u) * 16u;
+            for(int a = 0; a < 3; ++a){
+                uint32_t wl, wu;
+                if(RESUME){
+                    const uint32_t *w = (const uint32_t *) (sc.wnodes + (size_t) d.x * 4) + a * 4 + (d.y >> 1);
+                    wl = w[0]; wu = w[2];
+                } else {
+                    const uint32_t *w = (const uint32_t *) (sc.qnodes + (size_t) d.x * 2) + a * 2;
+                    wl = w[0]; wu = w[1];
+                }
+                lo[c][a] = (wl >> sh) & 0xFFFFu; hi[c][a] = (wu >> sh) & 0xFFFFu;
+            }
+        }
+        s_top[2 * threadIdx.x] = make_uint4(lo[0][0] | lo[1][0] << 16, hi[0][0] | hi[1][0] << 16, lo[0][1] | lo[1][1] << 16, hi[0][1] | hi[1][1] << 16);
+        s_top[2 * threadIdx.x + 1] = make_uint4(lo[0][2] | lo[1][2] << 16, hi[0][2] | hi[1][2] << 16, code[0], code[1]);
+        uint32_t *sw = (uint32_t *) (s_top + kRootWide);
+        sw[2 * threadIdx.x] = start[0]; sw[2 * threadIdx.x + 1] = start[1];
+        if(threadIdx.x == 0) sw[kRootWide] = RESUME ? 0u : sc.root_treelet[2 * kRootWide].x;
     }
     uint32_t ecount = ecount_ptr ? *ecount_ptr : 0u, scount = scount_ptr ? *scount_ptr : 0u;
     uint32_t ce = ecount >= kTraceShortQueue ? chunk_rays : (uint32_t) kBlock;
diff --git a/path_tracing_amd/csrc/scene_build.cpp b/path_tracing_amd/csrc/scene_build.cpp
--- a/path_tracing_amd/csrc/scene_build.cpp
+++ b/path_tracing_amd/csrc/scene_build.cpp
@@ -584,6 +584,51 @@
     quantise_tree(hs);
     pack_wide_boxes(hs);
     return "";
+}
+
+static void derive_root_treelets(HostScene &hs){
+    hs.root_binary.clear(); hs.root_wide.clear();
+    if(hs.nodes.empty() || hs.nodes[0].left == kEmptyChild || hs.nodes[0].right == kEmptyChild) return;
+    auto binary_area = [&](uint32_t node_side){
+        const BvhNode &b = hs.nodes[node_side >> 1];
+        const float *mn = (node_side & 1u) ? b.rmin : b.lmin, *mx = (node_side & 1u) ? b.rmax : b.lmax;
+        float dx = mx[0] - mn[0], dy = mx[1] - mn[1], dz = mx[2] - mn[2];
+        return dx * dy + dy * dz + dz * dx;
+    };
+    auto largest_inner = [](const std::vector<RootChild> &list, auto area){
+        int best = -1; float ba = -1.0f;
+        for(size_t k = 0; k < list.size(); ++k) if(!(list[k].code & kLeafFlag)){ float a = area(list[k]); if(a > ba){ ba = a; best = (int) k; } }
+        return best;
+    };
+    {   auto open = [&](uint32_t idx, uint32_t depth){
+            const BvhNode &b = hs.nodes[idx];
+            if(b.left != kEmptyChild) hs.root_binary.push_back(RootChild{ idx, 0u, b.left, depth });
+            if(b.right != kEmptyChild) hs.root_binary.push_back(RootChild{ idx, 1u, b.right, depth });
+        };
+        open(0u, 1u);
+        while((int) hs.root_binary.size() < kRootWide){
+            int best = largest_inner(hs.root_binary, [&](const RootChild &c){ return binary_area(c.src * 2u + c.slot); });
+            if(best < 0) break;
+            const RootChild c = hs.root_binary[(size_t) best];
+            hs.root_binary.erase(hs.root_binary.begin() + best);
+            open(c.code, c.depth + 1u);
+        }
+    }
+    {   auto kids_of = [&](uint32_t idx){ int n = 0; for(int k = 0; k < 4; ++k) if(hs.wnodes[idx].w[12 + k] != kEmptyChild) ++n; return n; };
+        auto open = [&](uint32_t idx, uint32_t depth){
+            for(uint32_t k = 0; k < 4u; ++k) if(hs.wnodes[idx].w[12 + k] != kEmptyChild) hs.root_wide.push_back(RootChild{ idx, k, hs.wnodes[idx].w[12 + k], depth });
+        };
+        open(0u, 1u);
+        for(;;){
+            int best = largest_inner(hs.root_wide, [&](const RootChild &c){ return binary_area(hs.wide_src[(size_t) c.src * 4 + c.slot]); });
+            if(best < 0) break;
+            const RootChild c = hs.root_wide[(size_t) best];
+            if((int) hs.root_wide.size() - 1 + kids_of(c.code) > kRootWide) break;
+            hs.root_wide.erase(hs.root_wide.begin() + best);
+            open(c.code, c.depth + 1u);
+        }
+        if((int) hs.root_wide.size() > kRootWide || hs.root_wide.size() < 2) hs.root_wide.clear();
+    }
 }
 
 const char *build_host_scene(const void *lights_v, int nl, const void *spheres_v, int ns,
@@ -761,6 +806,7 @@
         pack_wide_boxes(hs);
     }
 
+    derive_root_treelets(hs);
     lap("wide");
     hs.tris.resize(nt);
     pod_vector<uint32_t> mat_of((size_t) nt);
```

Result: no change. 2525 Msamples/s (median of 2 runs) (+0.6%).
